# radhofan/Fairify

Hardware: AMD Instinct MI355X
Metric: % partitions verified + partitions/sec on AC suite at 1/2/4/8 MI355X (higher is better)
Workload: dtype fp32

## Files before the change

### fairify_amd/csrc/args.h

```cpp
#pragma once
#include "common.h"

#define FA_MAX_PA 8
#define FA_MAX_RA 8
#define FA_CMAX_PA 8
#define FA_MAX_SPLIT 6

struct BoundArgs {
  const float* flat;
  const float* lo;
  const float* hi;
  const uint8_t* dead_in;
  int R;
  int symbolic;
  int G;
  int stride;
  int wstride;
  int wfloats;
  float* out_lb;
  float* out_ub;
  float* Lc; float* L0; float* Le;
  float* Uc; float* U0; float* Ue;
  float* layer_lb;
  float* layer_ub;
  uint8_t* dead_out;
  int V;
  int npa;
  int pa_idx[FA_MAX_PA];
  const float* values;
  const int* node_part;
  const uint8_t* dead_part;
  int part_mod;
  unsigned long long fold;
  const int8_t* skip_status;
  const int* skip_part;
  int skip_signdef;
  const uint8_t* row_open;
  int open_mod;
  const int8_t* phase_in;
  uint8_t* infeas;
};

#define FA_MAX_ESC 4
struct EscSteps {
  int n;
  int budget[FA_MAX_ESC];
  int open[FA_MAX_ESC];
};

struct FwdArgs {
  const float* flat;
  const float* x;
  int B;
  const uint8_t* dead;
  float* out;
  int S;
};

struct AscentArgs {
  const float* flat;
  const float* lo;
  const float* hi;
  const float* x0;
  const float* f0;
  const int* q0;
  int P, K, iters;
  int V, npa;
  int pa_idx[FA_MAX_PA];
  const int64_t* values;
  int Pp;
  const int64_t* pairs;
  int nfree;
  int free_idx[64];
  uint8_t* found;
  float* wit_x;
  float* wit_xp;
  int S;
};

struct FalsifyArgs {
  const float* flat;
  const float* lo;
  const float* hi;
  const int64_t* pids;
  int P;
  int n_samples;
  int n_local;
  uint32_t seed;
  int V, npa;
  int pa_idx[FA_MAX_PA];
  const int64_t* values;
  int Pp;
  const int64_t* pairs;
  int walk_k, walk_steps;
  int K, iters;
  int nfree;
  int free_idx[64];
  uint8_t* found;
  float* wit_x;
  float* wit_xp;
  int8_t* how;
  int nra;
  int ra_idx[FA_MAX_RA];
  int tau;
  uint32_t dseed;
};

struct SimArgs {
  const float* flat;
  const float* lo;
  const float* hi;
  const int64_t* pids;
  int P;
  int n_samples;
  uint32_t seed;
  int V;
  int npa;
  int pa_idx[FA_MAX_PA];
  const int64_t* values;
  int Pp;
  const int64_t* pairs;
  int nra;
  int ra_idx[FA_MAX_RA];
  int tau;
  int* counts;
  uint8_t* found;
  float* wit_x;
  float* wit_xp;
  float* z0;
  int* keys;
  int split;
  int S;
  int regcount;
};

struct CertArgs {
  int Nn, n0, V, Pp, norient;
  const float *Lc, *L0, *Le, *Uc, *U0, *Ue;
  const float *Lcp, *L0p, *Lep, *Ucp, *U0p, *Uep;
  const float *olb, *oub, *olbp, *oubp;
  const float *xlo, *xhi, *xplo, *xphi;
  const int64_t* pairs;
  const int64_t* values;
  int npa;
  int pa_idx[FA_CMAX_PA];
  int nra;
  int ra_idx[FA_MAX_RA];
  float tau;
  const uint8_t* shared;
  float unit;
  float gmarg;
  float* gmin;
  float* tstar;
  uint8_t* open;
  float* score;
  int64_t* split_dim;
  float* cand_x;
  float* cand_xp;
  int64_t* cand_v;
  int64_t* cand_o;
  float* scores;
  uint8_t* leaf;
  int skip_closed;
  const int8_t* status;
  const int* part;
  int smear;
  const float* lay_lb;
  const float* lay_ub;
  int lay_N;
  const float* W0T;
  int n1;
};

struct SettleArgs {
  int P;
  int8_t* status;
  int* lvl_open;
  int* part_open;
  const int* part_nodes;
  int* nodes_start;
  int* prev_start;
  const int* counters_cur;
  int* counters_next;
  int* host_counts;
  int* pbudget;
  uint8_t* prob;
  int budget2;
  int max_open;
  EscSteps esc;
  int* done;
};

struct SplitArgs {
  int Nn, n0, relaxed, nra, V, Pp, norient;
  int ra_idx[FA_MAX_RA];
  float tau;
  const float *xlo, *xhi, *xplo, *xphi;
  const int* part;
  const uint8_t* open;
  const uint8_t* leaf;
  const float* scores;
  const float* cand_x;
  const float* cand_xp;
  const float* pe_lb;
  const float* pe_ub;
  const float *olb, *oub, *olbp, *oubp;
  const int64_t* pairs;
  const int64_t* values;
  int npa;
  int pa_idx[FA_CMAX_PA];
  const uint8_t* shared;
  int8_t* status;
  int* part_nodes;
  int* part_open;
  int* lvl_open;
  const int* nodes_start;
  const int* prev_start;
  int budget;
  const int* pbudget;
  uint8_t* prob;
  int budget2;
  int m;
  int target;
  float *oxlo, *oxhi, *oxplo, *oxphi;
  int* opart;
  int* count_out;
  int cap;
  float* cand_buf;
  int* cand_count;
  int cand_cap;
  SettleArgs settle;
};

struct BabInitArgs {
  int P, n_run, n0;
  const unsigned char* stage;
  int8_t* status;
  int *nodes, *open_left, *lvl_open, *nodes_start, *prev_start;
  int* part;
  float *xlo, *xhi, *xplo, *xphi;
  int nra;
  int ra_idx[FA_MAX_RA];
  float tau;
  int* counters;
  int* pbudget;
  uint8_t* prob;
  int budget;
};

#define FA_DECODE_MAX_DIMS 64
struct DecodeDesc {
  int n0;
  int radix[FA_DECODE_MAX_DIMS];
  long long div[FA_DECODE_MAX_DIMS];
  int chunk_off[FA_DECODE_MAX_DIMS];
  float base_lo[FA_DECODE_MAX_DIMS];
  float base_hi[FA_DECODE_MAX_DIMS];
};

struct CrownPhaseArgs {
  const float* flat;
  const float* lo;
  const float* hi;
  int R;
  const int8_t* phase;
  const float* layer_lb;
  const float* layer_ub;
  const uint8_t* infeas;
  float* out_lb;
  float* out_ub;
  float *Lc, *L0, *Le, *Uc, *U0, *Ue;
  int* split;
  float* score;
  float* low;
  const int8_t* skip_status;
  const int* skip_part;
};

struct ReluLevelArgs {
  int Nn, n0, nh;
  int npa;
  int pa_idx[FA_CMAX_PA];
  const int64_t* pairs;
  const float* values;
  int neg_from;
  const int* part;
  const int* pair;
  const float* xlo;
  const float* xhi;
  const int8_t* phase;
  float* rlo;
  float* rhi;
  int* rpart;
  const float* olb;
  const float* oub;
  const uint8_t* infeas;
  const float *Lc, *L0, *Le, *Uc, *U0, *Ue;
  const int* split;
  uint8_t* open;
  int* choice;
  int* idim;
  float* cpts;
  const float* pe_lb;
  const float* pe_ub;
  int8_t* status;
  int* part_nodes;
  const int* nodes_start;
  int budget;
  int* opart;
  int* opair;
  float* oxlo;
  float* oxhi;
  int8_t* ophase;
  int* count_out;
  int cap;
  float* cand_buf;
  int* cand_count;
  int cand_cap;
  float unit;
  float gmarg;
  int nra;
  int ra_idx[FA_MAX_RA];
  float tau;
  const float* xplo;
  const float* xphi;
  float* oxplo;
  float* oxphi;
};

struct BetaArgs {
  const float* flat;
  const float* wt;
  int R;
  int npa;
  int pa_idx[FA_MAX_PA];
  const float* lo;
  const float* hi;
  const float* va;
  const float* vb;
  const float* LBA;
  const float* UBA;
  const float* LBB;
  const float* UBB;
  const int8_t* phA;
  const int8_t* phB;
  float* par;
  float* t;
  float* scratch;
  int iters;
  float lr_a, lr_b, lr_t, decay;
  int lookahead;
  int beta_pos;
  int stall;
  int pgap;
  int wpb;
  int wt_lds;
  double* bound;
  int* split;
  float* xstar;
  float* binit;
  unsigned long long ramask;
  const float* plo;
  const float* phi;
  float* xpstar;
  float* gtie;
  float tau;
  const int8_t* osg;
  const uint8_t* skip;
  int ph_stride;
  int feas;
  const float* pgsum;
  const float* pgn;
  float* fpar;
  float* fgt;
  double* fval;
};

struct BetaPoolArgs {
  int N;
  int n0, nh, nn;
  int npa;
  int pa_idx[FA_MAX_PA];
  int nra;
  int ra_idx[FA_MAX_RA];
  float tau;
  int leaf;
  int warm_beta;
  int count;
  const int* part; const int* tree; const int8_t* osg;
  const float* lo; const float* hi; const float* plo; const float* phi;
  const float* va; const float* vb;
  float* LBA; float* UBA; float* LBB; float* UBB;
  const int8_t* ph; const float* par; const float* t; const float* gt;
  int8_t* status; int* part_nodes; int budget;
  int* tree_cnt;
  uint8_t* skip;
  float* rlo; float* rhi; int* rpart;
  const float* lay_lb; const float* lay_ub;
  const uint8_t* infeas;
  const double* bound; const int* split; const float* xstar; const float* xpstar; const float* binit;
  float* cpts;
  const float* pe_lb; const float* pe_ub;
  int* opart; int* otree; int8_t* oosg;
  float* olo; float* ohi; float* oplo; float* ophi; float* ova; float* ovb;
  float* oLBA; float* oUBA; float* oLBB; float* oUBB;
  int8_t* oph; float* opar; float* ot; float* ogt;
  int* count_out; int cap;
  int* nan_count;
  int* diag;
  int root;
  float* cand_buf; int* cand_count; int cand_cap;
};

#define FA_RATE_SLOTS 32
#define FA_RATE_MAX_V 32
#define FA_RATE_MAX_E 32
struct RateArgs {
  const float* flat;
  const float* lo;
  const float* hi;
  const int64_t* pids;
  int P;
  int n_samples;
  uint32_t seed;
  int V;
  int npa;
  int pa_idx[FA_MAX_PA];
  const int64_t* values;
  int Pp;
  const int64_t* pairs;
  int nra;
  int ra_idx[FA_MAX_RA];
  int tau;
  int E;
  int* flips;
  int* amb;
  int* amb_idx;
  int split;
};

#define FA_COUNT_MAX_VOL 65536
struct EnumArgs {
  const float* flat;
  const float* lo;
  const float* hi;
  int L;
  int V;
  int npa;
  int pa_idx[FA_MAX_PA];
  const int64_t* values;
  int Pp;
  const int64_t* pairs;
  int nra;
  int ra_idx[FA_MAX_RA];
  int tau;
  int E;
  int max_vol;
  int* cert;
  int* amb;
  int* amb_idx;
  int blocks;
};

struct CountArgs {
  int N, n0, V;
  int npa;
  int pa_idx[FA_MAX_PA];
  int nra;
  int ra_idx[FA_MAX_RA];
  float tau;
  const float* lo;
  const float* hi;
  const float* values;
  float* rlo;
  float* rhi;
  float* plo;
  float* phi;
  const int* part;
  const float *lx, *ux;
  const float *lxp, *uxp;
  int Pp;
  const int64_t* pairs;
  const float* score;
  long long leaf_points;
  uint8_t* code;
  long long* fair;
  long long* unfair;
  int* child_cnt;
  float* olo;
  float* ohi;
  int* opart;
  int cap;
  float* leaf_lo;
  float* leaf_hi;
  int* leaf_part;
  int leaf_cap;
  int* counters;
};
```

### fairify_amd/csrc/bab.hip

```cpp
#include <stdlib.h>

#include <algorithm>

#include "args.h"

#define ST_UNKNOWN 0
#define ST_SAT 1
#define ST_UNSAT 2
#define ST_RUNNING 3
#define ST_STOPPING 4

__device__ __forceinline__ void fa_stop(const SplitArgs& a, int p) { a.status[p] = ST_STOPPING; }

template <class DIMS>
__device__ __forceinline__ void fa_child_dim(const SplitArgs& a, const float* xl, const float* xh, const float* pl,
                                             const float* ph, const DIMS& dims, int m, int c, int d, float& lo,
                                             float& hi, float& plo, float& phi) {
  lo = xl[d]; hi = xh[d]; plo = pl[d]; phi = ph[d];
  for (int j = 0; j < m; ++j) {
    const int dd = dims[j];
    const bool up = (c >> j) & 1;
    if (dd == d) {
      const float mid = floorf(0.5f * (xl[d] + xh[d]));
      if (up) lo = mid + 1.f; else hi = mid;
      if (a.relaxed && a.shared[d]) { plo = lo; phi = hi; }
    } else if (dd == a.n0 + d) {
      const float mid = floorf(0.5f * (pl[d] + ph[d]));
      if (up) plo = mid + 1.f; else phi = mid;
    }
  }
  if (a.relaxed)
    for (int k = 0; k < a.nra; ++k)
      if (a.ra_idx[k] == d) {
        plo = fmaxf(plo, lo - a.tau);
        phi = fminf(phi, hi + a.tau);
        lo = fmaxf(lo, plo - a.tau);
        hi = fminf(hi, phi + a.tau);
      }
}

struct FaPackedDims {
  unsigned long long v;
  __device__ __forceinline__ int operator[](int j) const { return (int)((v >> (7 * j)) & 127ull); }
};

__device__ __forceinline__ void fa_wave_argmax(float& s, int& d) {
#pragma unroll
  for (int o = 32; o > 0; o >>= 1) {
    const float s2 = __shfl_xor(s, o);
    const int d2 = __shfl_xor(d, o);
    if (s2 > s || (s2 == s && d2 < d)) { s = s2; d = d2; }
  }
}

__device__ __forceinline__ void fa_group_argmax(float& s, int& d) {
#pragma unroll
  for (int o = 8; o > 0; o >>= 1) {
    const float s2 = __shfl_xor(s, o);
    const int d2 = __shfl_xor(d, o);
    if (s2 > s || (s2 == s && d2 < d)) { s = s2; d = d2; }
  }
}

__device__ __forceinline__ void fa_settle_counters(const SettleArgs& s) {
  const int c0 = __hip_atomic_load(&s.counters_cur[0], __ATOMIC_RELAXED, __HIP_MEMORY_SCOPE_AGENT);
  const int c1 = __hip_atomic_load(&s.counters_cur[1], __ATOMIC_RELAXED, __HIP_MEMORY_SCOPE_AGENT);
  __hip_atomic_store(&s.host_counts[0], c0, __ATOMIC_RELAXED, __HIP_MEMORY_SCOPE_SYSTEM);
  __hip_atomic_store(&s.host_counts[1], c1, __ATOMIC_RELAXED, __HIP_MEMORY_SCOPE_SYSTEM);
  s.counters_next[0] = 0;
  s.counters_next[1] = 0;
}

__device__ __forceinline__ void fa_settle_part(const SettleArgs& s, int p) {
  const int8_t st = s.status[p];
  if (st == ST_STOPPING) {
    s.status[p] = ST_UNKNOWN;
    if (s.part_open) s.part_open[p] = s.lvl_open[p];
  } else if (s.prob && s.prob[p] && st == ST_RUNNING) {
    const int cur = s.pbudget[p];
    int k = 0;
    while (k < s.esc.n && s.esc.budget[k] <= cur) ++k;
    const int thr = k == 0 ? s.max_open : s.esc.open[k - 1];
    if (s.lvl_open[p] <= thr) {
      s.pbudget[p] = k < s.esc.n ? s.esc.budget[k] : s.budget2;
    } else {
      s.status[p] = ST_UNKNOWN;
      if (s.part_open) s.part_open[p] = s.lvl_open[p];
    }
  }
  if (s.prob) s.prob[p] = 0;
  s.lvl_open[p] = 0;
  s.prev_start[p] = s.nodes_start[p];
  s.nodes_start[p] = s.part_nodes[p];
}

struct FaSplitPlan {
  unsigned long long fmask;
  unsigned long long dims;
  int m;
  int nchild;
  int ncand;
  int leaf;
  int part;
};

__device__ __forceinline__ bool fa_leaf_poss(const SplitArgs& a, int n, int t) {
  const int o = t / a.Pp, q = t - o * a.Pp;
  const size_t ri = (size_t)n * a.V + (int)a.pairs[2 * q], rj = (size_t)n * a.V + (int)a.pairs[2 * q + 1];
  return (o == 0) ? (a.olb[ri] < 0.f && a.oubp[rj] > 0.f) : (a.oub[ri] > 0.f && a.olbp[rj] < 0.f);
}

__device__ __forceinline__ int fa_wave_incl_scan(int v, int lane) {
#pragma unroll
  for (int o = 1; o < 64; o <<= 1) {
    const int u = __shfl_up(v, o);
    if (lane >= o) v += u;
  }
  return v;
}

#define FA_SPLIT_WAVES 8
#define FA_SPLIT_NPW 8
#define FA_SPLIT_NB (FA_SPLIT_WAVES * FA_SPLIT_NPW)
struct FaSplitLds {
  FaSplitPlan plan[FA_SPLIT_NB];
  int child_off[FA_SPLIT_NB], cand_off[FA_SPLIT_NB];
  int part[FA_SPLIT_NB], ns[FA_SPLIT_NB], ws[FA_SPLIT_NB], bud[FA_SPLIT_NB];
  float pe[FA_SPLIT_NB][4];
  int8_t st[FA_SPLIT_NB];
  uint8_t open[FA_SPLIT_NB], leaf[FA_SPLIT_NB];
  int last;
};

__device__ __forceinline__ void fa_split_fetch(const SplitArgs& a, FaSplitLds& sh, int nb) {
  if (threadIdx.x >= nb && threadIdx.x < FA_SPLIT_NB) sh.plan[threadIdx.x] = FaSplitPlan{0ull, 0ull, 0, 0, 0, 0, -1};
  if (threadIdx.x < nb) {
    const int t = threadIdx.x;
    const int n = blockIdx.x * nb + t;
    uint8_t op = 0;
    int p = 0;
    if (n < a.Nn) {
      op = a.open[n];
      p = a.part[n];
      sh.leaf[t] = a.leaf[n];
      sh.pe[t][0] = a.pe_lb[n];
      sh.pe[t][1] = a.pe_ub[n];
      sh.pe[t][2] = a.pe_lb[a.Nn + n];
      sh.pe[t][3] = a.pe_ub[a.Nn + n];
    }
    sh.open[t] = op;
    sh.part[t] = p;
    if (op) {
      sh.st[t] = a.status[p];
      sh.ns[t] = a.nodes_start[p];
      sh.ws[t] = a.nodes_start[p] - a.prev_start[p];
      sh.bud[t] = a.pbudget ? a.pbudget[p] : a.budget;
    }
  }
  __syncthreads();
}

__device__ __forceinline__ void fa_split_reserve(const SplitArgs& a, FaSplitLds& sh) {
  const int lane = threadIdx.x & 63;
  __syncthreads();
  if (threadIdx.x < 64) {
    const int c = sh.plan[lane].nchild, q = sh.plan[lane].ncand;
    const int ci = fa_wave_incl_scan(c, lane), qi = fa_wave_incl_scan(q, lane);
    int cb = 0, qb = 0;
    if (lane == 63) {
      if (ci) cb = atomicAdd(a.count_out, ci);
      if (qi) qb = atomicAdd(a.cand_count, qi);
    }
    cb = __shfl(cb, 63);
    qb = __shfl(qb, 63);
    sh.child_off[lane] = cb + ci - c;
    sh.cand_off[lane] = qb + qi - q;
    const int p = sh.plan[lane].part;
    const int o = p >= 0 ? 1 : 0;
    const int oi = fa_wave_incl_scan(o, lane);
    const int pprev = __shfl_up(p, 1), pnext = __shfl_down(p, 1);
    const unsigned long long heads = __ballot(lane == 0 || pprev != p);
    const bool tail = lane == 63 || pnext != p;
    const int h = 63 - __clzll(heads & (lane == 63 ? ~0ull : ((2ull << lane) - 1ull)));
    const int ci_b = __shfl(ci, h > 0 ? h - 1 : 0), oi_b = __shfl(oi, h > 0 ? h - 1 : 0);
    if (tail && p >= 0) {
      const int so = oi - (h > 0 ? oi_b : 0), sc = ci - (h > 0 ? ci_b : 0);
      if (so && a.lvl_open) atomicAdd(&a.lvl_open[p], so);
      if (sc) atomicAdd(&a.part_nodes[p], sc);
    }
  }
  __syncthreads();
}

__device__ __forceinline__ void fa_split_settle_tail(const SplitArgs& a, FaSplitLds& sh) {
  if (a.settle.P > 0) {
    __threadfence();
    __syncthreads();
    if (threadIdx.x == 0) sh.last = atomicAdd(a.settle.done, 1) == (int)gridDim.x - 1;
    __syncthreads();
    if (sh.last) {
      __threadfence();
      if (threadIdx.x == 0) fa_settle_counters(a.settle);
      for (int p = threadIdx.x; p < a.settle.P; p += blockDim.x) fa_settle_part(a.settle, p);
      if (threadIdx.x == 0) *a.settle.done = 0;
    }
  }
}

__device__ __forceinline__ void fa_split_write_leaf(const SplitArgs& a, int n, int p, int t, int slot) {
  const int n0 = a.n0;
  if (slot >= a.cand_cap) {
    fa_stop(a, p);
    return;
  }
  const float* xl = a.xlo + (size_t)n * n0;
  const float* xpl = a.relaxed ? a.xplo + (size_t)n * n0 : xl;
  const int o = t / a.Pp, q = t - o * a.Pp;
  const int vi = (int)a.pairs[2 * q], vj = (int)a.pairs[2 * q + 1];
  float* cbuf = a.cand_buf + (size_t)slot * (2 * n0 + 1);
  for (int d = 0; d < n0; ++d) {
    cbuf[d] = xl[d];
    cbuf[n0 + d] = xpl[d];
  }
  for (int k = 0; k < a.npa; ++k) {
    cbuf[a.pa_idx[k]] = (float)a.values[vi * a.npa + k];
    cbuf[n0 + a.pa_idx[k]] = (float)a.values[vj * a.npa + k];
  }
  cbuf[2 * n0] = __int_as_float(p);
}

template <int W>
__device__ __forceinline__ void fa_split_write_inner(const SplitArgs& a, const FaSplitPlan& pl, int n, int p, int slot,
                                                     int off, int li) {
  const int n0 = a.n0;
  const float* xl = a.xlo + (size_t)n * n0;
  const float* xh = a.xhi + (size_t)n * n0;
  const float* xpl = a.relaxed ? a.xplo + (size_t)n * n0 : xl;
  const float* xph = a.relaxed ? a.xphi + (size_t)n * n0 : xh;
  if (pl.ncand) {
    if (slot < a.cand_cap) {
      float* cbuf = a.cand_buf + (size_t)slot * (2 * n0 + 1);
      for (int d = li; d < 2 * n0 + 1; d += W)
        cbuf[d] = d < n0 ? a.cand_x[(size_t)n * n0 + d]
                         : (d < 2 * n0 ? a.cand_xp[(size_t)n * n0 + d - n0] : __int_as_float(p));
    }
  }
  if (pl.nchild == 0) return;
  if (off + pl.nchild > a.cap) {
    if (li == 0) fa_stop(a, p);
    const int lim = a.cap - off;
    for (int e = li; e < lim * n0; e += W) {
      const int r = e / n0, d = e - r * n0;
      const size_t o = (size_t)(off + r) * n0 + d;
      a.oxlo[o] = xl[d];
      a.oxhi[o] = xh[d];
      if (a.relaxed) { a.oxplo[o] = xpl[d]; a.oxphi[o] = xph[d]; }
    }
    for (int r = li; r < lim; r += W) a.opart[off + r] = p;
    return;
  }
  const FaPackedDims dims{pl.dims};
  for (int c = li; c < (1 << pl.m); c += W)
    if ((pl.fmask >> c) & 1ull) a.opart[off + __popcll(pl.fmask & ((1ull << c) - 1ull))] = p;
  const int dense = (pl.fmask & (pl.fmask + 1ull)) == 0ull;
  for (int e = li; e < pl.nchild * n0; e += W) {
    const int r = e / n0, d = e - r * n0;
    int c = r;
    if (!dense) {
      unsigned long long mm = pl.fmask;
      for (int t = 0; t < r; ++t) mm &= mm - 1ull;
      c = __ffsll((long long)mm) - 1;
    }
    float lo, hi, plo, phi;
    fa_child_dim(a, xl, xh, xpl, xph, dims, pl.m, c, d, lo, hi, plo, phi);
    const size_t o = (size_t)(off + r) * n0 + d;
    a.oxlo[o] = lo;
    a.oxhi[o] = hi;
    if (a.relaxed) {
      a.oxplo[o] = plo;
      a.oxphi[o] = phi;
    }
  }
}

__global__ void __launch_bounds__(64 * FA_SPLIT_WAVES) fa_split_kernel(SplitArgs a, int npw) {
  __shared__ FaSplitLds sh;
  const int lane = threadIdx.x & 63;
  const int wave = threadIdx.x >> 6;
  const int n0 = a.n0;
  const int npair = a.norient * a.Pp;
  const int nb = FA_SPLIT_WAVES * npw;
  fa_split_fetch(a, sh, nb);
  for (int i = 0; i < npw; ++i) {
    const int loc = wave * npw + i;
    const int n = blockIdx.x * nb + loc;
    FaSplitPlan pl{0ull, 0ull, 0, 0, 0, 0, -1};
    do {
      if (n >= a.Nn || !sh.open[loc]) break;
      const int p = sh.part[loc];
      const int8_t s0 = sh.st[loc];
      if (s0 != ST_RUNNING && s0 != ST_STOPPING) break;
      if (sh.leaf[loc]) {
        pl.leaf = 1;
        for (int t0 = 0; t0 < npair; t0 += 64)
          pl.ncand += __popcll(__ballot(t0 + lane < npair && fa_leaf_poss(a, n, t0 + lane)));
        break;
      }
      pl.part = p;
      {
        const float lbx = sh.pe[loc][0], ubx = sh.pe[loc][1];
        const float lbp = sh.pe[loc][2], ubp = sh.pe[loc][3];
        pl.ncand = ((lbx < 0.f && ubp > 0.f) || (ubx > 0.f && lbp < 0.f)) ? 1 : 0;
      }
      const float* sc = a.scores + (size_t)n * 2 * n0;
      int mreq = 1;
      {
        const int mmax = a.m < FA_MAX_SPLIT ? a.m : FA_MAX_SPLIT;
        const int w = sh.ws[loc];
        while (mreq < mmax && ((long long)w << (mreq + 1)) <= (long long)a.target) ++mreq;
      }
      const int d0 = lane, d1 = lane + 64;
      float s0v = (d0 < 2 * n0) ? sc[d0] : -1.f;
      float s1v = (d1 < 2 * n0) ? sc[d1] : -1.f;
      if (!(s0v > -0.5f)) s0v = -1.f;
      if (!(s1v > -0.5f)) s1v = -1.f;
      int dims[FA_MAX_SPLIT];
      int m = 0;
      for (int j = 0; j < mreq; ++j) {
        float sv = s0v >= s1v ? s0v : s1v;
        int d = s0v >= s1v ? d0 : d1;
        if (sv <= -0.5f) d = 0x7fffffff;
        fa_wave_argmax(sv, d);
        if (sv <= -0.5f) break;
        dims[m++] = d;
        if (d == d0) s0v = -1.f;
        if (d == d1) s1v = -1.f;
      }
      if (m == 0) break;
      {
        const int bud = sh.bud[loc];
        if (sh.ns[loc] >= bud) {
          if (a.prob && bud < a.budget2) {
            if (lane == 0) a.prob[p] = 1;
          } else {
            if (lane == 0) fa_stop(a, p);
            break;
          }
        }
      }
      const int k = 1 << m;
      const float* xl = a.xlo + (size_t)n * n0;
      const float* xh = a.xhi + (size_t)n * n0;
      const float* xpl = a.relaxed ? a.xplo + (size_t)n * n0 : xl;
      const float* xph = a.relaxed ? a.xphi + (size_t)n * n0 : xh;
      bool ok = lane < k;
      if (a.relaxed && ok)
        for (int d = 0; d < n0; ++d) {
          float lo, hi, plo, phi;
          fa_child_dim(a, xl, xh, xpl, xph, dims, m, lane, d, lo, hi, plo, phi);
          ok = ok && lo <= hi && plo <= phi;
        }
      pl.fmask = __ballot(ok);
      pl.nchild = __popcll(pl.fmask);
      pl.m = m;
      for (int j = 0; j < m; ++j) pl.dims |= (unsigned long long)dims[j] << (7 * j);
    } while (false);
    if (lane == 0) sh.plan[loc] = pl;
  }
  fa_split_reserve(a, sh);
  for (int i = 0; i < npw; ++i) {
    const int loc = wave * npw + i;
    const int n = blockIdx.x * nb + loc;
    const FaSplitPlan pl = sh.plan[loc];
    if (pl.ncand == 0 && pl.nchild == 0) continue;
    const int p = sh.part[loc];
    if (pl.leaf) {
      int slot0 = sh.cand_off[loc];
      for (int t0 = 0; t0 < npair; t0 += 64) {
        const int t = t0 + lane;
        const bool poss = t < npair && fa_leaf_poss(a, n, t);
        const unsigned long long bm = __ballot(poss);
        if (poss) {
          const int slot = slot0 + __popcll(bm & ((1ull << lane) - 1ull));
          fa_split_write_leaf(a, n, p, t, slot);
        }
        slot0 += __popcll(bm);
      }
      continue;
    }
    fa_split_write_inner<64>(a, pl, n, p, sh.cand_off[loc], sh.child_off[loc], lane);
  }
  fa_split_settle_tail(a, sh);
}

#define FA_SPLIT_GPW 4
#define FA_SPLIT_NPP (FA_SPLIT_NB / (FA_SPLIT_WAVES * FA_SPLIT_GPW))
__global__ void __launch_bounds__(64 * FA_SPLIT_WAVES) fa_split_group_kernel(SplitArgs a, int npp) {
  __shared__ FaSplitLds sh;
  const int lane = threadIdx.x & 63;
  const int wave = threadIdx.x >> 6;
  const int gl = lane & 15, grp = lane >> 4;
  const int n0 = a.n0;
  const int npair = a.norient * a.Pp;
  const int nb = FA_SPLIT_WAVES * FA_SPLIT_GPW * npp;
  const int mmax = a.m < FA_MAX_SPLIT ? a.m : FA_MAX_SPLIT;
  fa_split_fetch(a, sh, nb);
  for (int i = 0; i < npp; ++i) {
    const int loc = (wave * npp + i) * FA_SPLIT_GPW + grp;
    const int n = blockIdx.x * nb + loc;
    FaSplitPlan pl{0ull, 0ull, 0, 0, 0, 0, -1};
    bool act = n < a.Nn && sh.open[loc];
    const int p = sh.part[loc];
    if (act) {
      const int8_t s0 = sh.st[loc];
      act = s0 == ST_RUNNING || s0 == ST_STOPPING;
    }
    const bool lf = act && sh.leaf[loc];
    if (__ballot(lf)) {
      for (int t0 = 0; t0 < npair; t0 += 16) {
        const unsigned long long bm = __ballot(lf && t0 + gl < npair && fa_leaf_poss(a, n, t0 + gl));
        pl.ncand += __popcll((bm >> (16 * grp)) & 0xffffull);
      }
    }
    pl.leaf = lf ? 1 : 0;
    const bool inner = act && !lf;
    int mreq = 1;
    float s0v = -1.f, s1v = -1.f;
    const int d0 = gl, d1 = gl + 16;
    if (inner) {
      pl.part = p;
      const float lbx = sh.pe[loc][0], ubx = sh.pe[loc][1];
      const float lbp = sh.pe[loc][2], ubp = sh.pe[loc][3];
      pl.ncand = ((lbx < 0.f && ubp > 0.f) || (ubx > 0.f && lbp < 0.f)) ? 1 : 0;
      const int w = sh.ws[loc];
      while (mreq < mmax && ((long long)w << (mreq + 1)) <= (long long)a.target) ++mreq;
      const float* sc = a.scores + (size_t)n * 2 * n0;
      if (d0 < 2 * n0) s0v = sc[d0];
      if (d1 < 2 * n0) s1v = sc[d1];
      if (!(s0v > -0.5f)) s0v = -1.f;
      if (!(s1v > -0.5f)) s1v = -1.f;
    }
    int m = 0;
    bool more = inner;
#pragma unroll
    for (int j = 0; j < FA_MAX_SPLIT; ++j) {
      float sv = s0v >= s1v ? s0v : s1v;
      int d = s0v >= s1v ? d0 : d1;
      if (sv <= -0.5f) d = 0x7fffffff;
      fa_group_argmax(sv, d);
      more = more && j < mreq && sv > -0.5f;
      if (more) {
        pl.dims |= (unsigned long long)d << (7 * j);
        m = j + 1;
        if (d == d0) s0v = -1.f;
        if (d == d1) s1v = -1.f;
      }
    }
    bool split = inner && m > 0;
    if (split) {
      const int bud = sh.bud[loc];
      if (sh.ns[loc] >= bud) {
        if (a.prob && bud < a.budget2) {
          if (gl == 0) a.prob[p] = 1;
        } else {
          if (gl == 0) fa_stop(a, p);
          split = false;
        }
      }
    }
    {
      const FaPackedDims dims{pl.dims};
      const float* xl = a.xlo + (size_t)n * n0;
      const float* xh = a.xhi + (size_t)n * n0;
      const float* xpl = a.relaxed ? a.xplo + (size_t)n * n0 : xl;
      const float* xph = a.relaxed ? a.xphi + (size_t)n * n0 : xh;
      unsigned long long fmask = 0ull;
      for (int c0 = 0; c0 < (1 << (mmax > 1 ? mmax : 1)); c0 += 16) {
        const int c = c0 + gl;
        bool ok = split && c < (1 << m);
        if (a.relaxed && ok)
          for (int d = 0; d < n0; ++d) {
            float lo, hi, plo, phi;
            fa_child_dim(a, xl, xh, xpl, xph, dims, m, c, d, lo, hi, plo, phi);
            ok = ok && lo <= hi && plo <= phi;
          }
        const unsigned long long bm = __ballot(ok);
        fmask |= ((bm >> (16 * grp)) & 0xffffull) << c0;
      }
      if (split) {
        pl.fmask = fmask;
        pl.nchild = __popcll(fmask);
        pl.m = m;
      } else {
        pl.dims = 0ull;
      }
    }
    if (gl == 0) sh.plan[loc] = pl;
  }
  fa_split_reserve(a, sh);
  for (int i = 0; i < npp; ++i) {
    const int loc = (wave * npp + i) * FA_SPLIT_GPW + grp;
    const int n = blockIdx.x * nb + loc;
    const FaSplitPlan pl = sh.plan[loc];
    const bool any = pl.ncand != 0 || pl.nchild != 0;
    if (!__ballot(any)) continue;
    const int p = sh.part[loc];
    const bool lf = any && pl.leaf;
    if (__ballot(lf)) {
      int slot0 = sh.cand_off[loc];
      for (int t0 = 0; t0 < npair; t0 += 16) {
        const int t = t0 + gl;
        const bool poss = lf && t < npair && fa_leaf_poss(a, n, t);
        const unsigned long long bm = (__ballot(poss) >> (16 * grp)) & 0xffffull;
        if (poss) fa_split_write_leaf(a, n, p, t, slot0 + __popcll(bm & ((1ull << gl) - 1ull)));
        slot0 += __popcll(bm);
      }
    }
    if (any && !pl.leaf) fa_split_write_inner<16>(a, pl, n, p, sh.cand_off[loc], sh.child_off[loc], gl);
  }
  fa_split_settle_tail(a, sh);
}

__global__ void fa_bab_init_kernel(BabInitArgs a) {
  const int tid = blockIdx.x * FA_THREADS + threadIdx.x;
  const int nth = gridDim.x * FA_THREADS;
  const int8_t* st = reinterpret_cast<const int8_t*>(a.stage);
  const int* run = reinterpret_cast<const int*>(a.stage + ((a.P + 3) & ~3));
  const float* lo = reinterpret_cast<const float*>(run + a.n_run);
  const float* hi = lo + (size_t)a.n_run * a.n0;
  for (int p = tid; p < a.P; p += nth) {
    a.status[p] = st[p];
    a.nodes[p] = 0;
    a.open_left[p] = 0;
    a.lvl_open[p] = 0;
    a.nodes_start[p] = 0;
    a.prev_start[p] = -1;
    if (a.pbudget) a.pbudget[p] = a.budget;
    if (a.prob) a.prob[p] = 0;
  }
  for (int i = tid; i < a.n_run; i += nth) a.part[i] = run[i];
  const size_t ne = (size_t)a.n_run * a.n0;
  for (size_t e = tid; e < ne; e += nth) {
    a.xlo[e] = lo[e];
    a.xhi[e] = hi[e];
    if (a.xplo) {
      const int d = (int)(e % a.n0);
      bool r = false;
      for (int k = 0; k < a.nra; ++k) r |= a.ra_idx[k] == d;
      a.xplo[e] = r ? lo[e] - a.tau : lo[e];
      a.xphi[e] = r ? hi[e] + a.tau : hi[e];
    }
  }
  if (tid < 5) a.counters[tid] = 0;
}

__global__ void fa_bab_finish_kernel(int P, const int8_t* status, const int* nodes, const int* open_left, int* out) {
  const int p = blockIdx.x * FA_THREADS + threadIdx.x;
  if (p >= P) return;
  out[p] = status[p];
  out[P + p] = nodes[p];
  out[2 * P + p] = open_left[p];
}

__global__ void fa_mark_unknown_kernel(const int* part, int n, int8_t* status) {
  const int i = blockIdx.x * FA_THREADS + threadIdx.x;
  if (i >= n) return;
  const int p = part[i];
  if (status[p] == ST_RUNNING || status[p] == ST_STOPPING) status[p] = ST_UNKNOWN;
}

__global__ void fa_settle_kernel(SettleArgs s) {
  const int p = blockIdx.x * FA_THREADS + threadIdx.x;
  if (p == 0) fa_settle_counters(s);
  if (p < s.P) fa_settle_part(s, p);
}

__global__ void fa_set_status_kernel(const int* idx, int n, int8_t* status, int8_t v) {
  const int i = blockIdx.x * FA_THREADS + threadIdx.x;
  if (i < n) status[idx[i]] = v;
}

extern "C" int fa_split_launch(SplitArgs a, hipStream_t stream) {
  if (a.Nn <= 0) return 0;
  if (a.nra > FA_MAX_RA || a.npa > FA_CMAX_PA || a.n0 > 64) return -3;
  if (2 * a.n0 <= 32) {
    const char* e = getenv("FAIRIFY_SPLIT_GROUPS");
    if (!(e && *e == '0')) {
      int npp = FA_SPLIT_NPP;
      while (npp > 1 && (a.Nn + FA_SPLIT_WAVES * FA_SPLIT_GPW * npp - 1) / (FA_SPLIT_WAVES * FA_SPLIT_GPW * npp) < 1024)
        npp >>= 1;
      const int nbg = FA_SPLIT_WAVES * FA_SPLIT_GPW * npp;
      hipLaunchKernelGGL(fa_split_group_kernel, dim3((a.Nn + nbg - 1) / nbg), dim3(64 * FA_SPLIT_WAVES), 0, stream, a,
                         npp);
      return (int)hipGetLastError();
    }
  }
  int npw = FA_SPLIT_NPW;
  while (npw > 1 && (a.Nn + FA_SPLIT_WAVES * npw - 1) / (FA_SPLIT_WAVES * npw) < 1024) npw >>= 1;
  const int nb = FA_SPLIT_WAVES * npw;
  hipLaunchKernelGGL(fa_split_kernel, dim3((a.Nn + nb - 1) / nb), dim3(64 * FA_SPLIT_WAVES), 0, stream, a, npw);
  return (int)hipGetLastError();
}

extern "C" int fa_mark_unknown_launch(const int* part, int n, int8_t* status, hipStream_t stream) {
  if (n <= 0) return 0;
  hipLaunchKernelGGL(fa_mark_unknown_kernel, dim3((n + FA_THREADS - 1) / FA_THREADS), dim3(FA_THREADS), 0, stream,
                     part, n, status);
  return (int)hipGetLastError();
}

extern "C" int fa_set_status_launch(const int* idx, int n, int8_t* status, int8_t v, hipStream_t stream) {
  if (n <= 0) return 0;
  hipLaunchKernelGGL(fa_set_status_kernel, dim3((n + FA_THREADS - 1) / FA_THREADS), dim3(FA_THREADS), 0, stream, idx,
                     n, status, v);
  return (int)hipGetLastError();
}

extern "C" int fa_settle_launch(SettleArgs s, hipStream_t stream) {
  const int n = s.P > 0 ? s.P : 1;
  hipLaunchKernelGGL(fa_settle_kernel, dim3((n + FA_THREADS - 1) / FA_THREADS), dim3(FA_THREADS), 0, stream, s);
  return (int)hipGetLastError();
}

extern "C" int fa_bab_init_launch(BabInitArgs a, hipStream_t stream) {
  if (a.nra > FA_MAX_RA) return -3;
  const long long work = std::max<long long>(std::max(a.P, a.n_run), (long long)a.n_run * a.n0);
  const int blocks = (int)std::min<long long>((work + FA_THREADS - 1) / FA_THREADS + 1, 4096);
  hipLaunchKernelGGL(fa_bab_init_kernel, dim3(blocks), dim3(FA_THREADS), 0, stream, a);
  return (int)hipGetLastError();
}

extern "C" int fa_bab_finish_launch(int P, const int8_t* status, const int* nodes, const int* open_left, int* out,
                                    hipStream_t stream) {
  if (P <= 0) return 0;
  hipLaunchKernelGGL(fa_bab_finish_kernel, dim3((P + FA_THREADS - 1) / FA_THREADS), dim3(FA_THREADS), 0, stream, P,
                     status, nodes, open_left, out);
  return (int)hipGetLastError();
}
```

### fairify_amd/csrc/bab_runtime.cpp

```cpp
#include <hip/hip_runtime.h>
#include <pybind11/numpy.h>
#include <pybind11/pybind11.h>
#include <pybind11/stl.h>

#include <algorithm>
#include <chrono>
#include <cmath>
#include <cstring>
#include <stdexcept>
#include <utility>
#include <vector>

#include "runtime_host.h"

namespace py = pybind11;

extern "C" int fa_certify_launch(CertArgs a, hipStream_t stream);
extern "C" int fa_split_launch(SplitArgs a, hipStream_t stream);
extern "C" int fa_mark_unknown_launch(const int* part, int n, int8_t* status, hipStream_t stream);
extern "C" int fa_settle_launch(SettleArgs s, hipStream_t stream);
extern "C" int fa_crown_launch(const NetDesc& net, BoundArgs a, hipStream_t stream);
extern "C" int fa_refine_launch(const NetDesc& net, BoundArgs a, hipStream_t stream);
extern "C" int fa_backward_launch(const NetDesc& net, BoundArgs a, hipStream_t stream);
extern "C" int fa_refine_crown_launch(const NetDesc& net, BoundArgs a, hipStream_t stream);
extern "C" int fa_bab_init_launch(BabInitArgs a, hipStream_t stream);
extern "C" int fa_bab_finish_launch(int P, const int8_t* status, const int* nodes, const int* open_left, int* out,
                                    hipStream_t stream);

const NetDesc& fa_net_desc(py::handle net);

namespace {

using fa_mem::DevBuf;
using fa_rt::ck;
using fa_rt::ckl;

bool point_skip_closed() {
  static const bool v = [] {
    const char* e = getenv("FAIRIFY_POINT_SKIP_CLOSED");
    return !(e && e[0] == '0');
  }();
  return v;
}

bool cert_skip_closed() {
  static const bool v = [] {
    const char* e = getenv("FAIRIFY_CERT_SKIP_CLOSED");
    return !(e && e[0] == '0');
  }();
  return v;
}

bool fuse_settle() {
  static const bool v = [] {
    const char* e = getenv("FAIRIFY_FUSE_SETTLE");
    return e && e[0] == '1';
  }();
  return v;
}

bool skip_signdef() {
  static const bool v = [] {
    const char* e = getenv("FAIRIFY_REFINE_SKIP_SIGNDEF");
    return !(e && e[0] == '0');
  }();
  return v;
}

}

class BabRuntime {
 public:
  BabRuntime(py::handle net, uintptr_t flat, std::vector<int> pa, std::vector<float> values_f,
             std::vector<int64_t> values_i, std::vector<int64_t> pairs, std::vector<int> ra, float tau,
             std::vector<uint8_t> shared, int capacity, int batch_nodes, int cand_cap, double unit, bool crown,
             int split_target, int refine, bool smear, py::object keep)
      : net_(fa_net_desc(net)),
        flat_((const float*)flat),
        keep_(std::move(keep)),
        pa_(std::move(pa)),
        ra_(std::move(ra)),
        tau_(tau),
        cap_(capacity),
        batch_(batch_nodes),
        cand_cap_(cand_cap),
        unit_(unit),
        crown_(crown),
        refine_(crown ? refine : 0),
        smear_(smear),
        split_target_(std::max(2, split_target)),
        sink_(net_.dims[0]) {
    n0_ = net_.dims[0];
    npa_ = (int)pa_.size();
    if (npa_ == 0 || npa_ > FA_CMAX_PA || (int)ra_.size() > FA_MAX_RA) throw std::invalid_argument("bad PA/RA");
    V_ = (int)(values_i.size() / npa_);
    Pp_ = (int)(pairs.size() / 2);
    relaxed_ = !ra_.empty() && tau_ > 0;
    norient_ = relaxed_ ? 2 : 1;
    if ((int)shared.size() != n0_) throw std::invalid_argument("shared mask size");
    vals_f_.ensure(values_f.size());
    vals_i_.ensure(values_i.size());
    pairs_.ensure(pairs.size());
    shared_.ensure(shared.size());
    ck(hipMemcpy(vals_f_.p, values_f.data(), values_f.size() * sizeof(float), hipMemcpyHostToDevice), "cp");
    ck(hipMemcpy(vals_i_.p, values_i.data(), values_i.size() * sizeof(int64_t), hipMemcpyHostToDevice), "cp");
    ck(hipMemcpy(pairs_.p, pairs.data(), pairs.size() * sizeof(int64_t), hipMemcpyHostToDevice), "cp");
    ck(hipMemcpy(shared_.p, shared.data(), shared.size(), hipMemcpyHostToDevice), "cp");
    pool_[0] = pool_[1] = 0;
    const size_t R = (size_t)batch_ * V_;
    for (int s = 0; s < (relaxed_ ? 2 : 1); ++s) form_[s].ensure(R, n0_, net_.n_neurons, crown_ || smear_);
    const size_t Q = (size_t)Pp_ * norient_;
    gmin_.ensure(batch_ * Q);
    tstar_.ensure(batch_ * Q);
    open_.ensure(batch_);
    leaf_.ensure(batch_);
    score_.ensure(batch_);
    split_.ensure(batch_);
    cv_.ensure(batch_);
    co_.ensure(batch_);
    cand_.ensure((size_t)2 * batch_ * n0_);
    scores_.ensure((size_t)batch_ * 2 * n0_);
    pe_lb_.ensure(2 * (size_t)batch_);
    pe_ub_.ensure(2 * (size_t)batch_);
    sink_.ensure_cand(cand_cap_, kCandFloor);
    counters_.ensure(5);
    exact_ = fa_rt::make_exact(net_, flat_, pa_, relaxed_ ? ra_ : std::vector<int>(), tau_);
    if (smear_ && n0_ > 32) smear_ = false;
    if (smear_) {
      const int nm = n0_ <= 16 ? 16 : 32, n1 = net_.dims[1];
      std::vector<float> wt((size_t)n1 * nm, 0.f);
      for (int j = 0; j < n1; ++j)
        for (int i = 0; i < n0_; ++i)
          wt[(size_t)j * nm + i] = (float)std::fabs(exact_.w[(size_t)net_.w_off[0] + (size_t)i * n1 + j]);
      w0t_.ensure(wt.size());
      ck(hipMemcpy(w0t_.p, wt.data(), wt.size() * sizeof(float), hipMemcpyHostToDevice), "cp w0t");
    }
  }

  void set_fuse_settle(bool v) { fuse_settle_ = v; }

  py::tuple solve(py::array_t<float, py::array::c_style | py::array::forcecast> lo,
                  py::array_t<float, py::array::c_style | py::array::forcecast> hi,
                  py::array_t<int8_t, py::array::c_style | py::array::forcecast> status0, int budget,
                  double time_budget, uintptr_t dead_part, py::object confirm, uintptr_t stream_i,
                  bool native_exact, int budget2, int max_w, std::vector<std::pair<int, int>> esc_steps) {
    const bool inline_esc = budget2 > budget && max_w > 0;
    EscSteps esc{};
    for (const auto& bo : esc_steps)
      if (bo.first > (esc.n ? esc.budget[esc.n - 1] : budget) && bo.first < budget2 && esc.n < FA_MAX_ESC) {
        esc.budget[esc.n] = bo.first;
        esc.open[esc.n] = bo.second;
        ++esc.n;
      }
    hipStream_t st = (hipStream_t)stream_i;
    const auto t0 = std::chrono::steady_clock::now();
    const int P = (int)lo.shape(0);
    if (lo.ndim() != 2 || lo.shape(1) != n0_ || hi.shape(0) != P || status0.shape(0) != P)
      throw std::invalid_argument("solve: shape mismatch");
    status_.ensure(P);
    nodes_.ensure(P);
    open_left_.ensure(P);
    lvl_open_.ensure(P);
    nodes_start_.ensure(P);
    prev_start_.ensure(P);
    if (inline_esc) {
      pbudget_.ensure(P);
      prob_.ensure(P);
    }
    int slot = 0;
    const int8_t* hstatus = status0.data();
    std::vector<int> run;
    for (int p = 0; p < P; ++p)
      if (hstatus[p] == 3) run.push_back(p);
    if ((int)run.size() > cap_) throw std::invalid_argument("more partitions than pool capacity");
    ensure_pool(0, std::max<long long>((long long)run.size(), 1));
    const size_t nrun = run.size();
    const size_t st_bytes = (size_t)((P + 3) & ~3) + nrun * sizeof(int) + 2 * nrun * n0_ * sizeof(float);
    hstage_.ensure(st_bytes);
    stage_.ensure(st_bytes);
    {
      unsigned char* h = hstage_.p;
      std::memcpy(h, hstatus, P);
      int* hr = reinterpret_cast<int*>(h + ((P + 3) & ~3));
      std::memcpy(hr, run.data(), nrun * sizeof(int));
      float* hl = reinterpret_cast<float*>(hr + nrun);
      float* hh = hl + nrun * n0_;
      for (size_t i = 0; i < nrun; ++i)
        for (int d = 0; d < n0_; ++d) {
          hl[i * n0_ + d] = lo.data()[(size_t)run[i] * n0_ + d];
          hh[i * n0_ + d] = hi.data()[(size_t)run[i] * n0_ + d];
        }
    }
    ck(hipMemcpyAsync(stage_.p, hstage_.p, st_bytes, hipMemcpyHostToDevice, st), "cp stage");
    {
      BabInitArgs ia{};
      ia.P = P; ia.n_run = (int)nrun; ia.n0 = n0_;
      ia.stage = stage_.p;
      ia.status = status_.p; ia.nodes = nodes_.p; ia.open_left = open_left_.p; ia.lvl_open = lvl_open_.p;
      ia.nodes_start = nodes_start_.p; ia.prev_start = prev_start_.p;
      ia.part = part_[0].p; ia.xlo = lo_[0].p; ia.xhi = hi_[0].p;
      ia.xplo = relaxed_ ? plo_[0].p : nullptr; ia.xphi = relaxed_ ? phi_[0].p : nullptr;
      ia.nra = relaxed_ ? (int)ra_.size() : 0;
      for (int k = 0; k < ia.nra; ++k) ia.ra_idx[k] = ra_[k];
      ia.tau = tau_;
      ia.counters = counters_.p;
      ia.pbudget = inline_esc ? pbudget_.p : nullptr;
      ia.prob = inline_esc ? prob_.p : nullptr;
      ia.budget = budget;
      ckl(fa_bab_init_launch(ia, st), "bab_init");
    }
    int cur = 0;
    int n_in = (int)nrun;
    fa_exact::Witnesses wit(P, n0_, lo.data(), hi.data());
    hcount_.reset();
    int levels = 0, launches = 0, cand_overflow = 0;
    long long total_nodes = 0;
    bool timed_out = false;
    {
    py::gil_scoped_release nogil;
    while (n_in > 0) {
      const double el = std::chrono::duration<double>(std::chrono::steady_clock::now() - t0).count();
      if (el > time_budget) {
        ckl(fa_mark_unknown_launch(part_[cur].p, n_in, status_.p, st), "mark");
        timed_out = true;
        break;
      }
      int* cnt = counters_.p + 2 * slot;
      const int nxt = cur ^ 1;
      ensure_pool(nxt, 2LL * n_in + (long long)split_target_ * std::min(P, n_in));
      sink_.ensure_cand((long long)n_in * std::max(1, Pp_ * norient_), kCandFloor);
      SettleArgs se{};
      se.P = P; se.status = status_.p; se.lvl_open = lvl_open_.p; se.part_open = open_left_.p;
      se.part_nodes = nodes_.p; se.nodes_start = nodes_start_.p; se.prev_start = prev_start_.p;
      se.counters_cur = cnt; se.counters_next = counters_.p + 2 * (slot ^ 1); se.host_counts = hcount_.host_ptr();
      se.pbudget = inline_esc ? pbudget_.p : nullptr; se.prob = inline_esc ? prob_.p : nullptr;
      se.budget2 = budget2; se.max_open = max_w; se.esc = esc;
      se.done = counters_.p + 4;
      bool settled = false;
      for (int s = 0; s < n_in; s += batch_) {
        const int nb = std::min(batch_, n_in - s);
        const float* blo = lo_[cur].p + (size_t)s * n0_;
        const float* bhi = hi_[cur].p + (size_t)s * n0_;
        const float* bplo = relaxed_ ? plo_[cur].p + (size_t)s * n0_ : blo;
        const float* bphi = relaxed_ ? phi_[cur].p + (size_t)s * n0_ : bhi;
        const int* bpart = part_[cur].p + s;
        launch_bounds(blo, bhi, bpart, nb, 0, dead_part, st);
        if (relaxed_) launch_bounds(bplo, bphi, bpart, nb, 1, dead_part, st);
        const int sx = relaxed_ ? 1 : 0;
        CertArgs c{};
        c.Nn = nb; c.n0 = n0_; c.V = V_; c.Pp = Pp_; c.norient = norient_;
        const fa_rt::FormBufs &fx = form_[0], &fp = form_[sx];
        c.Lc = fx.Lc.p; c.L0 = fx.L0.p; c.Le = fx.Le.p; c.Uc = fx.Uc.p; c.U0 = fx.U0.p; c.Ue = fx.Ue.p;
        c.Lcp = fp.Lc.p; c.L0p = fp.L0.p; c.Lep = fp.Le.p; c.Ucp = fp.Uc.p; c.U0p = fp.U0.p; c.Uep = fp.Ue.p;
        c.olb = fx.olb.p; c.oub = fx.oub.p; c.olbp = fp.olb.p; c.oubp = fp.oub.p;
        c.xlo = blo; c.xhi = bhi; c.xplo = bplo; c.xphi = bphi;
        c.pairs = pairs_.p; c.values = vals_i_.p; c.npa = npa_;
        for (int k = 0; k < npa_; ++k) c.pa_idx[k] = pa_[k];
        c.nra = relaxed_ ? (int)ra_.size() : 0;
        for (int k = 0; k < c.nra; ++k) c.ra_idx[k] = ra_[k];
        c.tau = tau_;
        c.shared = shared_.p;
        c.unit = (float)unit_;
        c.gmarg = fa_rt::gamma_up(2 * n0_ + 4, unit_);
        c.gmin = gmin_.p; c.tstar = tstar_.p;
        c.open = open_.p; c.score = score_.p; c.split_dim = split_.p;
        c.cand_x = cand_.p; c.cand_xp = cand_.p + (size_t)nb * n0_;
        c.cand_v = cv_.p; c.cand_o = co_.p;
        c.scores = scores_.p; c.leaf = leaf_.p;
        if (cert_skip_closed()) { c.skip_closed = 1; c.status = status_.p; c.part = bpart; }
        if (smear_ && !relaxed_) {
          c.smear = 1;
          c.lay_lb = fx.lay_lb.p; c.lay_ub = fx.lay_ub.p; c.lay_N = net_.n_neurons;
          c.W0T = w0t_.p; c.n1 = net_.dims[1];
        }
        ckl(fa_certify_launch(c, st), "certify");
        fa_rt::screen_points(net_, flat_, cand_.p, 2 * nb, pe_lb_.p, pe_ub_.p, st, bpart, nb,
                             (const uint8_t*)dead_part, point_skip_closed() ? open_.p : nullptr, nb);
        SplitArgs sa{};
        sa.Nn = nb; sa.n0 = n0_; sa.relaxed = relaxed_ ? 1 : 0; sa.nra = relaxed_ ? (int)ra_.size() : 0;
        for (int k = 0; k < sa.nra; ++k) sa.ra_idx[k] = ra_[k];
        sa.V = V_; sa.Pp = Pp_; sa.norient = norient_; sa.tau = tau_;
        sa.xlo = blo; sa.xhi = bhi; sa.xplo = bplo; sa.xphi = bphi; sa.part = bpart;
        sa.open = open_.p; sa.leaf = leaf_.p; sa.scores = scores_.p;
        sa.cand_x = c.cand_x; sa.cand_xp = c.cand_xp; sa.pe_lb = pe_lb_.p; sa.pe_ub = pe_ub_.p;
        sa.olb = c.olb; sa.oub = c.oub; sa.olbp = c.olbp; sa.oubp = c.oubp;
        sa.pairs = pairs_.p; sa.values = vals_i_.p; sa.npa = npa_;
        for (int k = 0; k < npa_; ++k) sa.pa_idx[k] = pa_[k];
        sa.shared = shared_.p;
        sa.status = status_.p; sa.part_nodes = nodes_.p; sa.part_open = open_left_.p; sa.lvl_open = lvl_open_.p;
        sa.nodes_start = nodes_start_.p;
        sa.prev_start = prev_start_.p;
        sa.budget = budget; sa.m = FA_MAX_SPLIT; sa.target = split_target_;
        sa.pbudget = inline_esc ? pbudget_.p : nullptr;
        sa.prob = inline_esc ? prob_.p : nullptr;
        sa.budget2 = budget2;
        sa.oxlo = lo_[nxt].p; sa.oxhi = hi_[nxt].p;
        sa.oxplo = relaxed_ ? plo_[nxt].p : nullptr; sa.oxphi = relaxed_ ? phi_[nxt].p : nullptr;
        sa.opart = part_[nxt].p; sa.count_out = cnt; sa.cap = pool_[nxt];
        sa.cand_buf = sink_.records(); sa.cand_count = cnt + 1; sa.cand_cap = sink_.cand_alloc_;
        if (s + nb >= n_in && fuse_settle_) {
          sa.settle = se;
          settled = true;
        }
        ckl(fa_split_launch(sa, st), "split");
        launches += (relaxed_ ? 2 : 1) * (refine_ == 2 ? 1 : 2) + 3;
      }
      if (!settled) {
        ckl(fa_settle_launch(se, st), "settle");
        ++launches;
      }
      ck(hipStreamSynchronize(st), "sync");
      slot ^= 1;
      total_nodes += n_in;
      const int n_out = std::min(hcount_.children(), pool_[nxt]);
      const int n_cand_all = hcount_.candidates();
      const int n_cand = std::min(n_cand_all, sink_.cand_alloc_);
      if (n_cand_all > sink_.cand_alloc_) ++cand_overflow;
      ++levels;
      if (n_cand > 0)
        sink_.confirm_candidates(n_cand, wit, native_exact ? &exact_ : nullptr, confirm, status_.p, st);
      cur = nxt;
      n_in = n_out;
    }
    }
    out_.ensure((size_t)3 * P);
    hout_.ensure((size_t)3 * P * sizeof(int));
    ckl(fa_bab_finish_launch(P, status_.p, nodes_.p, open_left_.p, out_.p, st), "bab_finish");
    ck(hipMemcpyAsync(hout_.p, out_.p, (size_t)3 * P * sizeof(int), hipMemcpyDeviceToHost, st), "cp out");
    ck(hipStreamSynchronize(st), "sync");
    const int* hres = reinterpret_cast<const int*>(hout_.p);
    py::array_t<int8_t> status_out(P);
    py::array_t<int64_t> nodes_out(P), open_out(P);
    for (int p = 0; p < P; ++p) {
      int8_t v = (int8_t)hres[p];
      if (wit.got[p]) v = 1;
      else if (v == 3) v = timed_out ? 0 : 2;
      status_out.mutable_data()[p] = v;
      nodes_out.mutable_data()[p] = hres[P + p];
      open_out.mutable_data()[p] = (v == 0) ? hres[2 * P + p] : 0;
    }
    const double el = std::chrono::duration<double>(std::chrono::steady_clock::now() - t0).count();
    py::dict stats;
    stats["levels"] = levels;
    stats["launches"] = launches;
    stats["cand_overflow_levels"] = cand_overflow;
    stats["nodes"] = total_nodes;
    stats["time"] = el;
    stats["timed_out"] = timed_out;
    py::array_t<int64_t> ax({P, n0_}), axp({P, n0_});
    std::memcpy(ax.mutable_data(), wit.cex_x.data(), sizeof(int64_t) * wit.cex_x.size());
    std::memcpy(axp.mutable_data(), wit.cex_xp.data(), sizeof(int64_t) * wit.cex_xp.size());
    stats["open_left"] = open_out;
    return py::make_tuple(status_out, ax, axp, nodes_out, stats);
  }

 private:
  void launch_bounds(const float* lo, const float* hi, const int* part, int nb, int slot, uintptr_t dead_part,
                     hipStream_t st) {
    BoundArgs b{};
    b.flat = flat_;
    b.lo = lo;
    b.hi = hi;
    b.R = nb * V_;
    b.symbolic = 1;
    form_[slot].fill(b);
    b.V = V_;
    b.npa = npa_;
    for (int k = 0; k < npa_; ++k) b.pa_idx[k] = pa_[k];
    b.values = vals_f_.p;
    if (dead_part) {
      b.node_part = part;
      b.dead_part = (const uint8_t*)dead_part;
    }
    b.skip_status = status_.p;
    b.skip_part = part;
    if (refine_ == 2) {
      if (smear_) { b.layer_lb = form_[slot].lay_lb.p; b.layer_ub = form_[slot].lay_ub.p; }
      const int rc = fa_backward_launch(net_, b, st);
      if (rc == 0) return;
      if (rc != -1) ckl(rc, "backward");
      refine_ = 1;
    }
    if (crown_ || smear_) {
      b.layer_lb = form_[slot].lay_lb.p;
      b.layer_ub = form_[slot].lay_ub.p;
    }
    ckl(fa_bounds_launch(net_, b, st), "bounds");
    if (refine_ == 1) {
      b.skip_signdef = (!relaxed_ && npa_ == 1 && Pp_ == V_ * (V_ - 1) && skip_signdef()) ? 1 : 0;
      const int rc = fa_refine_crown_launch(net_, b, st);
      if (rc == 0) return;
      if (rc != -1) ckl(rc, "refine");
      refine_ = 0;
    }
    if (crown_) {
      const int rc = fa_crown_launch(net_, b, st);
      if (rc == -1) crown_ = false;
      else ckl(rc, "crown");
    }
  }

  void ensure_pool(int i, long long need) {
    const int want = (int)std::min<long long>(std::max<long long>(need, 1), cap_);
    if (want <= pool_[i]) return;
    const int n = fa_rt::grow_to(pool_[i], want, 1 << 16, cap_);
    const size_t cn = (size_t)n * n0_;
    lo_[i].ensure(cn);
    hi_[i].ensure(cn);
    part_[i].ensure(n);
    if (relaxed_) {
      plo_[i].ensure(cn);
      phi_[i].ensure(cn);
    }
    pool_[i] = n;
  }

  NetDesc net_;
  const float* flat_;
  py::object keep_;
  fa_exact::ExactChecker exact_;
  std::vector<int> pa_, ra_;
  float tau_;
  int cap_, batch_, cand_cap_;
  static constexpr int kCandFloor = 1 << 16;
  int pool_[2] = {0, 0};
  double unit_;
  bool crown_ = false;
  int refine_ = 0;
  bool smear_ = false;
  bool fuse_settle_ = fuse_settle();
  int split_target_ = 256;
  int n0_ = 0, npa_ = 0, V_ = 0, Pp_ = 0, norient_ = 1;
  bool relaxed_ = false;
  DevBuf<float> vals_f_, w0t_;
  DevBuf<int64_t> vals_i_, pairs_;
  DevBuf<uint8_t> shared_;
  DevBuf<float> lo_[2], hi_[2], plo_[2], phi_[2];
  DevBuf<int> part_[2];
  fa_rt::FormBufs form_[2];
  DevBuf<float> gmin_, tstar_, score_, cand_, scores_, pe_lb_, pe_ub_;
  DevBuf<uint8_t> open_, leaf_;
  DevBuf<int64_t> split_, cv_, co_;
  DevBuf<int> counters_, nodes_, open_left_, lvl_open_, nodes_start_, prev_start_, out_, pbudget_;
  DevBuf<int8_t> status_;
  DevBuf<uint8_t> prob_;
  DevBuf<unsigned char> stage_;
  fa_rt::LevelCounters hcount_;
  fa_mem::HostBuf hstage_, hout_;
  fa_rt::CandSink sink_;
};

void register_bab(py::module& m) {
  py::class_<BabRuntime>(m, "BabRuntime")
      .def(py::init<py::handle, uintptr_t, std::vector<int>, std::vector<float>, std::vector<int64_t>,
                    std::vector<int64_t>, std::vector<int>, float, std::vector<uint8_t>, int, int, int, double, bool,
                    int, int, bool, py::object>(),
           py::arg("net"), py::arg("flat"), py::arg("pa"), py::arg("values_f"), py::arg("values_i"),
           py::arg("pairs"), py::arg("ra"), py::arg("tau"), py::arg("shared"), py::arg("capacity"),
           py::arg("batch_nodes"), py::arg("cand_cap"), py::arg("unit"), py::arg("crown") = true,
           py::arg("split_target") = 256, py::arg("refine") = 0, py::arg("smear") = false, py::arg("keep") = py::none())
      .def("set_fuse_settle", &BabRuntime::set_fuse_settle, py::arg("on"))
      .def("solve", &BabRuntime::solve, py::arg("lo"), py::arg("hi"), py::arg("status"), py::arg("budget"),
           py::arg("time_budget"), py::arg("dead_part"), py::arg("confirm"), py::arg("stream"),
           py::arg("native_exact") = false, py::arg("budget2") = 0, py::arg("max_w") = 0,
           py::arg("esc_steps") = std::vector<std::pair<int, int>>{});
}
```

### fairify_amd/csrc/bindings.cpp

```cpp
#include <hip/hip_runtime.h>
#include <pybind11/pybind11.h>
#include <pybind11/stl.h>

#include <algorithm>
#include <cmath>
#include <cstring>
#include <cstdint>
#include <stdexcept>
#include <vector>

#include "kwargs.h"
#include "runtime_host.h"

extern "C" int fa_bounds_launch(const NetDesc& net, BoundArgs args, hipStream_t stream);
extern "C" int fa_crown_phase_launch(const NetDesc& net, CrownPhaseArgs a, hipStream_t stream);
extern "C" size_t fa_crown_phase_bytes(const NetDesc& net);
extern "C" int fa_point_try_launch(const NetDesc& net, BoundArgs a, hipStream_t stream);
extern "C" int fa_forward_launch(const NetDesc& net, FwdArgs a, hipStream_t stream);
extern "C" int fa_sim_launch(const NetDesc& net, SimArgs a, hipStream_t stream);
extern "C" int fa_sim_shaped(const NetDesc& net);
extern "C" int fa_rate_launch(const NetDesc& net, RateArgs a, hipStream_t stream);
extern "C" int fa_count_enum_launch(const NetDesc& net, EnumArgs a, hipStream_t stream);
extern "C" int fa_count_rows_launch(CountArgs a, hipStream_t stream);
extern "C" int fa_count_level_launch(CountArgs a, hipStream_t stream);
extern "C" int fa_ascent_launch(const NetDesc& net, AscentArgs a, hipStream_t stream);
extern "C" int fa_certify_launch(CertArgs a, hipStream_t stream);
extern "C" int fa_falsify_launch(const NetDesc& net, FalsifyArgs a, hipStream_t stream);
extern "C" int fa_prune_masks_launch(const NetDesc& net, int P, const int* counts, const float* ub, int ub_stride,
                                     const uint8_t* sym_dead, uint8_t* code, int* cnt, hipStream_t stream);
extern "C" int fa_heuristic_launch(const NetDesc& net, int Pu, const int64_t* rows, const float* lb, const float* ub,
                                   int stride, const uint8_t* code, double q50, double qlo, double qhi, uint8_t* hnew,
                                   uint8_t* hmerged, int* hcnt, hipStream_t stream);
extern "C" int fa_agree_launch(const NetDesc& net, const float* flat, int Pm, const int64_t* rows, const float* lo,
                               const float* hi, const int64_t* pids, const uint8_t* dead, int S, uint32_t seed,
                               int* agree, hipStream_t stream);

extern "C" int fa_decode_launch(const DecodeDesc& d, const int64_t* ids, int P, const float* chunk_lo,
                                const float* chunk_hi, float* lo, float* hi, hipStream_t stream);
extern "C" int fa_trace_marker_launch(int tag, int* sink, hipStream_t stream);
extern "C" int fa_beta_launch(const NetDesc& nd, BetaArgs a, hipStream_t stream);
extern "C" int fa_beta_config(const NetDesc& nd, int* wpb, int* wtl, size_t* bytes);
extern "C" int fa_beta_opt16_fits(const NetDesc& nd);
extern "C" size_t fa_beta_opt16_scratch_floats(const NetDesc& nd, int R);
extern "C" int fa_beta_opt16_launch(const NetDesc& nd, BetaArgs a, float* pgsum, float* pgn, hipStream_t stream);
extern "C" int fa_beta_level16_launch(const NetDesc& nd, BetaArgs a, hipStream_t stream);
extern "C" int fa_beta_opt16_feas_launch(const NetDesc& nd, BetaArgs a, hipStream_t stream);
extern "C" int fa_beta_feas16_launch(const NetDesc& nd, BetaArgs a, hipStream_t stream);
extern "C" int fa_knn_launch(const float* X, int n, int d, int k, int* idx, float* dist, hipStream_t stream);
extern "C" int fa_actdiff_launch(const NetDesc& net, const float* flat, const float* x, const float* xp, int npairs,
                                 float* sum_out, hipStream_t stream);
extern "C" int fa_pack_masks_launch(const uint8_t* src, int P, int N, int stride, int sel, uint8_t* out, int NB,
                                    unsigned long long* hash, hipStream_t stream);

template <typename T>
static T* P(uintptr_t p) { return reinterpret_cast<T*>(p); }

using fa_rt::gamma_up;

struct Net {
  NetDesc d;
  explicit Net(const std::vector<int>& dims, double unit) {
    if (dims.size() < 2 || dims.size() > FA_MAX_LAYERS + 1) throw std::invalid_argument("bad layer count");
    std::memset(&d, 0, sizeof(d));
    d.n_layers = (int)dims.size() - 1;
    int off = 0, noff = 0, mw = 0, mws = 0;
    for (size_t i = 0; i < dims.size(); ++i) {
      d.dims[i] = dims[i];
      mw = std::max(mw, dims[i]);
    }
    for (int l = 0; l < d.n_layers; ++l) {
      d.w_off[l] = off;
      off += dims[l] * dims[l + 1];
      d.b_off[l] = off;
      off += dims[l + 1];
      d.neuron_off[l] = noff;
      noff += dims[l + 1];
      mws = std::max(mws, dims[l] * dims[l + 1]);
      d.g_gemm[l] = gamma_up(2 * dims[l] + 1, unit);
      d.g_fwd[l] = gamma_up(dims[l] + 1, unit);
    }
    d.n_neurons = noff;
    d.n_hidden = noff - dims.back();
    d.max_width = mw;
    d.max_wsize = mws;
    d.unit = (float)unit;
    d.g_conc = gamma_up(dims[0] + 1, unit);
    d.g_one = gamma_up(1, unit);
    n_params = off;
    d.wperm_off = (off + 3) & ~3;
    int wp = 0;
    for (int l = 0; l < d.n_layers; ++l) wp += ((dims[l] + 15) / 16) * ((dims[l + 1] + 15) / 16) * 256;
    for (int l = 0; l < d.n_layers; ++l) wp += dims[l + 1];
    d.wperm_floats = (wp + 3) & ~3;
    total_floats = d.wperm_off + d.wperm_floats;
    d.pack_g = 1;
    if (d.n_layers >= 2 && dims[0] <= 16 && mw <= 16) {
      int mh = 0;
      for (int l = 1; l < d.n_layers; ++l) mh = std::max(mh, dims[l]);
      d.pack_g = mh <= 4 ? 4 : (mh <= 8 ? 2 : 1);
    }
    d.pack_off = total_floats;
    d.pack_floats = 0;
    if (d.pack_g > 1) {
      d.pack_floats = d.pack_g * 256 + (d.n_layers - 1) * 256 + d.n_layers * 16;
      total_floats += d.pack_floats;
    }
    d.wback_off = total_floats;
    int wb = 0;
    for (int l = 0; l < d.n_layers; ++l) wb += ((dims[l] + 15) / 16) * ((dims[l + 1] + 15) / 16) * 256;
    d.wback_floats = wb;
    total_floats += wb;
  }
  int n_params;
  int total_floats;
};

const NetDesc& fa_net_desc(py::handle h) { return h.cast<const Net&>().d; }
void register_bab(py::module& m);
void register_relu(py::module& m);
void register_beta(py::module& m);
extern "C" int fa_crown_launch(const NetDesc& net, BoundArgs a, hipStream_t stream);
extern "C" int fa_refine_launch(const NetDesc& net, BoundArgs a, hipStream_t stream);
extern "C" int fa_backward_launch(const NetDesc& net, BoundArgs a, hipStream_t stream);
extern "C" int fa_refine_crown_launch(const NetDesc& net, BoundArgs a, hipStream_t stream);
void register_csv(py::module& m);

using fa_rt::ckl;

static hipStream_t finish(Kw& k) {
  const hipStream_t s = reinterpret_cast<hipStream_t>(k.u64("stream"));
  k.done();
  return s;
}

static int dims(Kw& k, const char* key, int* idx, size_t cap, const char* too_many) {
  const std::vector<int> v = k.ints(key);
  if (v.size() > cap) throw std::invalid_argument(too_many);
  std::copy(v.begin(), v.end(), idx);
  return (int)v.size();
}

enum { OUT = 1, FORMS = 2, LAYERS = 4 };
template <typename A>
static A row_args(Kw& k, int req, const char* lo = "lo", const char* hi = "hi") {
  auto p = [&](const char* key, int group) { return (req & group) ? k.need<float>(key) : k.ptr<float>(key); };
  A a{};
  a.flat = k.need<const float>("flat");
  a.lo = k.need<const float>(lo);
  a.hi = k.need<const float>(hi);
  a.R = k.i("R");
  a.out_lb = p("out_lb", OUT);
  a.out_ub = p("out_ub", OUT);
  a.Lc = p("Lc", FORMS); a.L0 = p("L0", FORMS); a.Le = p("Le", FORMS);
  a.Uc = p("Uc", FORMS); a.U0 = p("U0", FORMS); a.Ue = p("Ue", FORMS);
  a.layer_lb = p("layer_lb", LAYERS);
  a.layer_ub = p("layer_ub", LAYERS);
  return a;
}
static BoundArgs bound_args(Kw& k, int req, const char* lo = "lo", const char* hi = "hi") {
  BoundArgs a = row_args<BoundArgs>(k, req, lo, hi);
  a.dead_in = k.ptr<const uint8_t>("dead_in");
  return a;
}

template <typename A>
static void fill_query(A& a, Kw& k, const char* too_many) {
  a.flat = k.need<const float>("flat");
  a.lo = k.need<const float>("lo");
  a.hi = k.need<const float>("hi");
  a.P = k.i("P");
  a.V = k.i("V");
  a.npa = dims(k, "pa", a.pa_idx, FA_MAX_PA, too_many);
  a.values = k.ptr<const int64_t>("values");
  a.Pp = k.i("Pp");
  a.pairs = k.ptr<const int64_t>("pairs");
}
template <typename A>
static void fill_samples(A& a, Kw& k, const char* too_many) {
  a.pids = k.need<const int64_t>("pids");
  a.n_samples = k.i("n_samples");
  a.seed = (uint32_t)k.u64("seed");
  a.nra = dims(k, "ra", a.ra_idx, FA_MAX_RA, too_many);
  a.tau = k.i("tau");
}
template <typename A>
static void fill_ascent(A& a, Kw& k, const char* too_many) {
  a.K = k.i("K");
  a.iters = k.i("iters");
  a.nfree = dims(k, "free", a.free_idx, 64, too_many);
  a.found = k.need<uint8_t>("found");
  a.wit_x = k.need<float>("wit_x");
  a.wit_xp = k.need<float>("wit_xp");
}

static BetaArgs beta_args(const Net& net, Kw& k) {
  BetaArgs a;
  std::memset(&a, 0, sizeof(a));
  a.flat = k.need<const float>("flat");
  a.wt = k.ptr<const float>("wt");
  a.R = k.i("R");
  a.npa = dims(k, "pa", a.pa_idx, FA_MAX_PA, "beta_level: too many PA dims");
  for (int q = 0; q < a.npa; ++q)
    if (a.pa_idx[q] < 0 || a.pa_idx[q] >= net.d.dims[0] || (q && a.pa_idx[q] <= a.pa_idx[q - 1]))
      throw std::invalid_argument("beta_level: PA dims must be increasing input indices");
  a.lo = k.need<const float>("lo");
  a.hi = k.need<const float>("hi");
  a.va = k.need<const float>("va");
  a.vb = k.need<const float>("vb");
  a.LBA = k.need<const float>("LBA");
  a.UBA = k.need<const float>("UBA");
  a.LBB = k.need<const float>("LBB");
  a.UBB = k.need<const float>("UBB");
  a.phA = k.need<const int8_t>("phA");
  a.phB = k.need<const int8_t>("phB");
  a.par = k.need<float>("par");
  a.t = k.need<float>("t");
  a.scratch = k.need<float>("scratch");
  a.iters = k.i("iters");
  a.lr_a = k.f("lr_a");
  a.lr_b = k.f("lr_b");
  a.lr_t = k.f("lr_t");
  a.decay = k.f("decay");
  a.lookahead = k.i("lookahead", 0);
  a.beta_pos = k.i("beta_pos", 1);
  const int flags = k.i("flags", 0);
  a.stall = flags & 1;
  a.pgap = (flags >> 1) & 3;
  a.feas = (flags >> 3) & 1;
  a.bound = k.ptr<double>("bound");
  a.split = k.ptr<int>("split");
  a.xstar = k.ptr<float>("xstar");
  a.binit = k.ptr<float>("binit");
  a.ramask = k.u64("ramask", 0);
  a.plo = k.ptr<const float>("plo");
  a.phi = k.ptr<const float>("phi");
  a.xpstar = k.ptr<float>("xpstar");
  a.gtie = k.ptr<float>("gtie");
  a.tau = k.f("tau", 0.f);
  a.osg = k.ptr<const int8_t>("osg");
  a.pgsum = k.ptr<const float>("pgsum");
  a.pgn = k.ptr<const float>("pgn");
  a.fpar = k.ptr<float>("fpar");
  a.fgt = k.ptr<float>("fgt");
  a.fval = k.ptr<double>("fval");
  if ((net.d.dims[0] < 64 && (a.ramask >> net.d.dims[0])) || (a.ramask && (!a.plo || !a.phi)))
    throw std::invalid_argument("beta_level: RA mask beyond the inputs or no x' box");
  return a;
}

PYBIND11_MODULE(_C, m) {
  m.doc() = "fairify_amd CDNA4 (gfx950) kernels";
  py::class_<Net>(m, "Net")
      .def(py::init<const std::vector<int>&, double>())
      .def_readonly("n_params", &Net::n_params)
      .def_readonly("total_floats", &Net::total_floats)
      .def_property_readonly("wperm_off", [](const Net& n) { return n.d.wperm_off; })
      .def_property_readonly("pack_g", [](const Net& n) { return n.d.pack_g; })
      .def_property_readonly("pack_off", [](const Net& n) { return n.d.pack_off; })
      .def_property_readonly("n_hidden", [](const Net& n) { return n.d.n_hidden; })
      .def_property_readonly("n_neurons", [](const Net& n) { return n.d.n_neurons; });

  m.def("bounds", [](const Net& net, py::kwargs kw) {
    Kw k("bounds", kw);
    const int symbolic = k.i("symbolic");
    BoundArgs a = bound_args(k, symbolic ? OUT | FORMS : OUT);
    a.symbolic = symbolic;
    a.G = k.i("G", 0);
    a.dead_out = k.ptr<uint8_t>("dead_out");
    a.fold = k.u64("fold", 0);
    a.phase_in = k.ptr<const int8_t>("phase_in");
    a.infeas = k.ptr<uint8_t>("infeas");
    ckl(fa_bounds_launch(net.d, a, finish(k)), "bounds");
  });

  m.def("crown_phase", [](const Net& net, py::kwargs kw) {
    Kw k("crown_phase", kw);
    CrownPhaseArgs a = row_args<CrownPhaseArgs>(k, OUT | FORMS | LAYERS);
    a.phase = k.ptr<const int8_t>("phase");
    a.infeas = k.ptr<const uint8_t>("infeas");
    a.split = k.need<int>("split");
    a.score = k.need<float>("score");
    a.low = k.ptr<float>("low");
    const int rc = fa_crown_phase_launch(net.d, a, finish(k));
    if (rc != 0) throw std::runtime_error("crown_phase launch failed, code " + std::to_string(rc));
  });

  m.def("relu_fits", [](const Net& net) { return fa_crown_phase_bytes(net.d) > 0; });

  m.def("crown", [](const Net& net, py::kwargs kw) {
    Kw k("crown", kw);
    const BoundArgs a = bound_args(k, OUT | FORMS | LAYERS);
    ckl(fa_crown_launch(net.d, a, finish(k)), "crown");
  });

  m.def("refine", [](const Net& net, py::kwargs kw) {
    Kw k("refine", kw);
    BoundArgs a = bound_args(k, LAYERS);
    a.phase_in = k.ptr<const int8_t>("phase_in");
    a.infeas = k.ptr<uint8_t>("infeas");
    const int rc = fa_refine_launch(net.d, a, finish(k));
    if (rc < -1) throw std::runtime_error("refine launch failed, code " + std::to_string(rc));
    return rc;
  });
  m.def("refine_crown", [](const Net& net, py::kwargs kw) {
    Kw k("refine_crown", kw);
    const BoundArgs a = bound_args(k, OUT | FORMS | LAYERS);
    const int rc = fa_refine_crown_launch(net.d, a, finish(k));
    if (rc < -1) throw std::runtime_error("refine_crown launch failed, code " + std::to_string(rc));
    return rc;
  });
  m.def("backward_bounds", [](const Net& net, py::kwargs kw) {
    Kw k("backward_bounds", kw);
    const BoundArgs a = bound_args(k, OUT | FORMS);
    const int rc = fa_backward_launch(net.d, a, finish(k));
    if (rc < -1) throw std::runtime_error("backward_bounds launch failed, code " + std::to_string(rc));
    return rc;
  });

  m.def("point_bounds", [](const Net& net, py::kwargs kw) {
    Kw k("point_bounds", kw);
    BoundArgs a = bound_args(k, OUT, "x", "x");
    a.row_open = k.ptr<const uint8_t>("row_open");
    a.open_mod = k.i("open_mod", 0);
    if (a.row_open && a.open_mod <= 0) throw std::invalid_argument("point_bounds: row_open needs open_mod > 0");
    const hipStream_t stream = finish(k);
    const int rc = fa_point_try_launch(net.d, a, stream);
    if (rc < 0) ckl(-rc, "point_bounds");
    if (rc == 0) ckl(fa_bounds_launch(net.d, a, stream), "point_bounds(ibp)");
  });

  m.def("forward", [](const Net& net, uintptr_t flat, uintptr_t x, int B, uintptr_t dead, uintptr_t out,
                      uintptr_t stream) {
    FwdArgs a{};
    a.flat = P<const float>(flat);
    a.x = P<const float>(x);
    a.B = B;
    a.dead = P<const uint8_t>(dead);
    a.out = P<float>(out);
    ckl(fa_forward_launch(net.d, a, (hipStream_t)stream), "forward");
  });

  m.def("sim", [](const Net& net, py::kwargs kw) {
    Kw k("sim", kw);
    SimArgs a{};
    fill_query(a, k, "too many PA/RA dims");
    fill_samples(a, k, "too many PA/RA dims");
    a.counts = k.need<int>("counts");
    a.found = k.need<uint8_t>("found");
    a.wit_x = k.need<float>("wit_x");
    a.wit_xp = k.need<float>("wit_xp");
    a.z0 = k.ptr<float>("z0");
    a.keys = k.ptr<int>("keys");
    a.split = k.i("split");
    a.regcount = k.i("regcount");
    if (a.split < 1 || (a.split > 1 && !a.keys)) throw std::invalid_argument("sim: split > 1 needs a keys buffer");
    ckl(fa_sim_launch(net.d, a, finish(k)), "sim");
  });
  m.def("sim_shaped", [](const Net& net) { return fa_sim_shaped(net.d) != 0; });

  m.def("rate", [](const Net& net, py::kwargs kw) {
    Kw k("rate", kw);
    RateArgs a{};
    fill_query(a, k, "too many PA/RA dims");
    fill_samples(a, k, "too many PA/RA dims");
    a.E = k.i("E");
    a.flips = k.need<int>("flips");
    a.amb = k.need<int>("amb");
    a.amb_idx = k.need<int>("amb_idx");
    a.split = k.i("split");
    const int rc = fa_rate_launch(net.d, a, finish(k));
    if (rc == -3) throw std::invalid_argument("rate: shape not covered (layer > 160, inputs > 32, V > 32 or E > 32)");
    ckl(rc, "rate");
  });

  m.def("count_enum", [](const Net& net, py::kwargs kw) {
    Kw k("count_enum", kw);
    EnumArgs a{};
    a.flat = k.need<const float>("flat");
    a.lo = k.need<const float>("lo");
    a.hi = k.need<const float>("hi");
    a.L = k.i("L");
    a.V = k.i("V");
    a.npa = dims(k, "pa", a.pa_idx, FA_MAX_PA, "too many PA/RA dims");
    a.values = k.need<const int64_t>("values");
    a.Pp = k.i("Pp");
    a.pairs = k.ptr<const int64_t>("pairs");
    a.nra = dims(k, "ra", a.ra_idx, FA_MAX_RA, "too many PA/RA dims");
    a.tau = k.i("tau");
    a.E = k.i("E");
    a.max_vol = k.i("max_vol");
    a.cert = k.need<int>("cert");
    a.amb = k.need<int>("amb");
    a.amb_idx = k.need<int>("amb_idx");
    a.blocks = k.i("blocks");
    if (a.Pp > 0 && !a.pairs) throw py::type_error("count_enum() missing required keyword argument 'pairs'");
    const int rc = fa_count_enum_launch(net.d, a, finish(k));
    if (rc == -3)
      throw std::invalid_argument(
          "count_enum: shape not covered (layer > 160, inputs > 32, V > 32, E > 32 or leaf volume > 65536)");
    ckl(rc, "count_enum");
  });
  auto count_args = [](Kw& k) {
    CountArgs a{};
    a.N = k.i("N");
    a.n0 = k.i("n0");
    a.V = k.i("V");
    a.npa = dims(k, "pa", a.pa_idx, FA_MAX_PA, "too many PA/RA dims");
    a.lo = k.need<const float>("lo");
    a.hi = k.need<const float>("hi");
    return a;
  };
  m.def("count_rows", [count_args](py::kwargs kw) {
    Kw k("count_rows", kw);
    CountArgs a = count_args(k);
    a.nra = dims(k, "ra", a.ra_idx, FA_MAX_RA, "too many PA/RA dims");
    a.tau = k.f("tau");
    a.values = k.need<const float>("values");
    a.rlo = k.need<float>("rlo");
    a.rhi = k.need<float>("rhi");
    a.plo = k.ptr<float>("plo");
    a.phi = k.ptr<float>("phi");
    ckl(fa_count_rows_launch(a, finish(k)), "count_rows");
  });
  m.def("count_level", [count_args](py::kwargs kw) {
    Kw k("count_level", kw);
    CountArgs a = count_args(k);
    a.part = k.need<const int>("part");
    a.lx = k.need<const float>("lx");
    a.ux = k.need<const float>("ux");
    a.lxp = k.need<const float>("lxp");
    a.uxp = k.need<const float>("uxp");
    a.Pp = k.i("Pp");
    a.pairs = k.ptr<const int64_t>("pairs");
    a.score = k.need<const float>("score");
    a.leaf_points = (long long)k.u64("leaf_points");
    a.code = k.need<uint8_t>("code");
    a.fair = k.need<long long>("fair");
    a.unfair = k.need<long long>("unfair");
    a.child_cnt = k.need<int>("child_cnt");
    a.olo = k.need<float>("olo");
    a.ohi = k.need<float>("ohi");
    a.opart = k.need<int>("opart");
    a.cap = k.i("cap");
    a.leaf_lo = k.need<float>("leaf_lo");
    a.leaf_hi = k.need<float>("leaf_hi");
    a.leaf_part = k.need<int>("leaf_part");
    a.leaf_cap = k.i("leaf_cap");
    a.counters = k.need<int>("counters");
    if (a.Pp > 0 && !a.pairs) throw py::type_error("count_level() missing required keyword argument 'pairs'");
    ckl(fa_count_level_launch(a, finish(k)), "count_level");
  });

  m.def("ascent", [](const Net& net, py::kwargs kw) {
    Kw k("ascent", kw);
    AscentArgs a{};
    fill_query(a, k, "too many PA/free dims");
    fill_ascent(a, k, "too many PA/free dims");
    a.x0 = k.need<const float>("x0");
    a.f0 = k.need<const float>("f0");
    a.q0 = k.need<const int>("q0");
    const int rc = fa_ascent_launch(net.d, a, finish(k));
    if (rc == -1) return false;
    ckl(rc, "ascent");
    return true;
  });

  m.def("falsify", [](const Net& net, py::kwargs kw) {
    Kw k("falsify", kw);
    FalsifyArgs a{};
    fill_query(a, k, "too many PA/RA/free dims");
    fill_samples(a, k, "too many PA/RA/free dims");
    fill_ascent(a, k, "too many PA/RA/free dims");
    if (a.tau <= 0) {
      a.nra = 0;
      std::fill_n(a.ra_idx, FA_MAX_RA, 0);
    }
    a.n_local = k.i("n_local");
    a.walk_k = k.i("walk_k");
    a.walk_steps = k.i("walk_steps");
    a.how = k.need<int8_t>("how");
    a.dseed = (uint32_t)k.u64("dseed");
    const int rc = fa_falsify_launch(net.d, a, finish(k));
    if (rc == 0) return false;
    if (rc < 0) ckl(-rc, "falsify");
    return true;
  });


  m.def("prune_masks", [](const Net& net, int Pn, uintptr_t counts, uintptr_t ub, int ub_stride, uintptr_t sym_dead,
                          uintptr_t code, uintptr_t cnt, uintptr_t stream) {
    ckl(fa_prune_masks_launch(net.d, Pn, P<const int>(counts), P<const float>(ub), ub_stride,
                                P<const uint8_t>(sym_dead), P<uint8_t>(code), P<int>(cnt), (hipStream_t)stream),
          "prune_masks");
  });

  m.def("heuristic", [](const Net& net, int Pu, uintptr_t rows, uintptr_t lb, uintptr_t ub, int stride, uintptr_t code,
                        double q50, double qlo, double qhi, uintptr_t hnew, uintptr_t hmerged, uintptr_t hcnt,
                        uintptr_t stream) {
    ckl(fa_heuristic_launch(net.d, Pu, P<const int64_t>(rows), P<const float>(lb), P<const float>(ub), stride,
                              P<const uint8_t>(code), q50, qlo, qhi, P<uint8_t>(hnew), P<uint8_t>(hmerged),
                              P<int>(hcnt), (hipStream_t)stream),
          "heuristic");
  });

  m.def("agree", [](const Net& net, uintptr_t flat, int Pm, uintptr_t rows, uintptr_t lo, uintptr_t hi, uintptr_t pids,
                    uintptr_t dead, int S, uint32_t seed, uintptr_t agree, uintptr_t stream) {
    const int rc = fa_agree_launch(net.d, P<const float>(flat), Pm, P<const int64_t>(rows), P<const float>(lo),
                                   P<const float>(hi), P<const int64_t>(pids), P<const uint8_t>(dead), S, seed,
                                   P<int>(agree), (hipStream_t)stream);
    if (rc == 0) return false;
    if (rc < 0) ckl(-rc, "agree");
    return true;
  });

  m.def("certify", [](py::kwargs kw) {
    Kw k("certify", kw);
    auto in = [&](const char* key) { return k.need<const float>(key); };
    CertArgs a{};
    a.Nn = k.i("Nn"); a.n0 = k.i("n0"); a.V = k.i("V"); a.Pp = k.i("Pp"); a.norient = k.i("norient");
    a.Lc = in("Lc"); a.L0 = in("L0"); a.Le = in("Le"); a.Uc = in("Uc"); a.U0 = in("U0"); a.Ue = in("Ue");
    a.olb = in("olb"); a.oub = in("oub");
    a.Lcp = in("Lcp"); a.L0p = in("L0p"); a.Lep = in("Lep"); a.Ucp = in("Ucp"); a.U0p = in("U0p"); a.Uep = in("Uep");
    a.olbp = in("olbp"); a.oubp = in("oubp");
    a.xlo = in("xlo"); a.xhi = in("xhi"); a.xplo = in("xplo"); a.xphi = in("xphi");
    a.pairs = k.ptr<const int64_t>("pairs");
    a.values = k.ptr<const int64_t>("values");
    a.npa = dims(k, "pa", a.pa_idx, FA_CMAX_PA, "too many PA/RA dims");
    a.nra = dims(k, "ra", a.ra_idx, FA_MAX_RA, "too many PA/RA dims");
    a.tau = k.f("tau");
    a.shared = k.need<const uint8_t>("shared");
    a.unit = k.f("unit");
    a.gmarg = std::nextafter(k.f("gmarg"), INFINITY);
    a.gmin = k.ptr<float>("gmin"); a.tstar = k.ptr<float>("tstar");
    a.open = k.need<uint8_t>("open"); a.score = k.need<float>("score"); a.split_dim = k.need<int64_t>("split_dim");
    a.cand_x = k.need<float>("cand_x"); a.cand_xp = k.need<float>("cand_xp");
    a.cand_v = k.need<int64_t>("cand_v"); a.cand_o = k.need<int64_t>("cand_o");
    a.scores = k.ptr<float>("scores"); a.leaf = k.ptr<uint8_t>("leaf");
    ckl(fa_certify_launch(a, finish(k)), "certify");
  });

  m.def("decode", [](std::vector<int> radix, std::vector<long long> div, std::vector<int> chunk_off,
                     std::vector<float> base_lo, std::vector<float> base_hi, uintptr_t ids, int Pn,
                     uintptr_t chunk_lo, uintptr_t chunk_hi, uintptr_t lo, uintptr_t hi, uintptr_t stream) {
    const size_t n0 = radix.size();
    if (n0 == 0 || n0 > FA_DECODE_MAX_DIMS || div.size() != n0 || chunk_off.size() != n0 || base_lo.size() != n0 ||
        base_hi.size() != n0)
      throw std::invalid_argument("decode: descriptor sizes");
    DecodeDesc d{};
    d.n0 = (int)n0;
    for (size_t k = 0; k < n0; ++k) {
      if (radix[k] < 0 || (radix[k] > 0 && div[k] <= 0)) throw std::invalid_argument("decode: radix/div");
      d.radix[k] = radix[k];
      d.div[k] = div[k];
      d.chunk_off[k] = chunk_off[k];
      d.base_lo[k] = base_lo[k];
      d.base_hi[k] = base_hi[k];
    }
    ckl(fa_decode_launch(d, P<const int64_t>(ids), Pn, P<const float>(chunk_lo), P<const float>(chunk_hi),
                           P<float>(lo), P<float>(hi), (hipStream_t)stream),
          "decode");
  });
  m.def("pack_masks", [](uintptr_t src, int Pn, int N, int stride, int sel, uintptr_t out, int NB, uintptr_t hash,
                         uintptr_t stream) {
    ckl(fa_pack_masks_launch(P<const uint8_t>(src), Pn, N, stride, sel, P<uint8_t>(out), NB,
                               P<unsigned long long>(hash), (hipStream_t)stream),
          "pack_masks");
  });
  m.def("knn", [](uintptr_t X, int n, int d, int k, uintptr_t idx, uintptr_t dist, uintptr_t stream) {
    ckl(fa_knn_launch(P<const float>(X), n, d, k, P<int>(idx), P<float>(dist), (hipStream_t)stream), "knn");
  });
  m.def("actdiff", [](const Net& net, uintptr_t flat, uintptr_t x, uintptr_t xp, int npairs, uintptr_t sum_out,
                      uintptr_t stream) {
    ckl(fa_actdiff_launch(net.d, P<const float>(flat), P<const float>(x), P<const float>(xp), npairs,
                            P<float>(sum_out), (hipStream_t)stream),
          "actdiff");
  });
  m.def("trace_marker", [](int tag, uintptr_t sink, uintptr_t stream) {
    ckl(fa_trace_marker_launch(tag, P<int>(sink), (hipStream_t)stream), "trace_marker");
  });
  m.def("beta_level", [](const Net& net, py::kwargs kw) {
    Kw k("beta_level", kw);
    const BetaArgs a = beta_args(net, k);
    return fa_beta_launch(net.d, a, finish(k));
  });
  m.def("beta_level16", [](const Net& net, py::kwargs kw) {
    Kw k("beta_level16", kw);
    const BetaArgs a = beta_args(net, k);
    return fa_beta_level16_launch(net.d, a, finish(k));
  });
  m.def("beta_opt16", [](const Net& net, py::kwargs kw) {
    Kw k("beta_opt16", kw);
    BetaArgs a = beta_args(net, k);
    float* pgsum = const_cast<float*>(a.pgsum);
    float* pgn = const_cast<float*>(a.pgn);
    a.wt = a.pgsum = a.pgn = nullptr;
    return fa_beta_opt16_launch(net.d, a, pgsum, pgn, finish(k));
  });
  m.def("beta_feas", [](const Net& net, py::kwargs kw) {
    Kw k("beta_feas", kw);
    BetaArgs a = beta_args(net, k);
    const int mode = k.i("mode");
    const hipStream_t st = finish(k);
    if (mode < 0 || mode > 3) throw std::invalid_argument("beta_feas: mode must be 0..3");
    if (mode != 0 && !a.fpar) throw std::invalid_argument("beta_feas: fpar required");
    a.lookahead = a.stall = a.pgap = 0;
    a.beta_pos = a.feas = 1;
    a.split = nullptr;
    a.xstar = a.binit = a.xpstar = nullptr;
    if (mode == 0) {
      a.fpar = a.fgt = nullptr;
      return fa_beta_launch(net.d, a, st);
    }
    if (mode == 1) return fa_beta_feas16_launch(net.d, a, st);
    if (mode == 2) return fa_beta_opt16_feas_launch(net.d, a, st);
    a.iters = 0;
    return fa_beta_launch(net.d, a, st);
  });
  m.def("beta_batched_fits", [](const Net& net) { return fa_beta_opt16_fits(net.d) != 0; });
  m.def("beta_opt16_scratch", [](const Net& net, int R) { return fa_beta_opt16_scratch_floats(net.d, R); });
  m.def("beta_config", [](const Net& net) {
    int w = 0, t = 0;
    size_t b = 0;
    const int rc = fa_beta_config(net.d, &w, &t, &b);
    return py::make_tuple(rc, w, t, b);
  });
  m.def("beta_fits", [](const Net& net) {
    int w = 0, t = 0;
    size_t b = 0;
    return fa_beta_config(net.d, &w, &t, &b) == 0;
  });
  m.def("arch", []() { return std::string("gfx950"); });
  m.def("prepare_lds", [] { return fa_lds_prepare(); });
  m.def("lds_registered", [] { return (int)fa_lds_registry().size(); });
  register_bab(m);
  register_relu(m);
  register_beta(m);
  m.def("mem_stats", [] {
    const fa_mem::Stats s = fa_mem::stats();
    py::dict d;
    d["dev_cached_bytes"] = s.dev_cached_bytes;
    d["dev_live_bytes"] = s.dev_live_bytes;
    d["host_cached_bytes"] = s.host_cached_bytes;
    d["host_live_bytes"] = s.host_live_bytes;
    d["dev_mallocs"] = s.dev_mallocs;
    d["dev_hits"] = s.dev_hits;
    d["host_mallocs"] = s.host_mallocs;
    d["host_hits"] = s.host_hits;
    d["driver_frees"] = s.driver_frees;
    return d;
  });
  m.def("mem_release_cached", [] { fa_mem::release_cached(); });
  register_csv(m);
}
```

### fairify_amd/csrc/certify.hip

```cpp
#include "args.h"

struct Form {
  const float* c;
  float c0;
  float fmag;
};

__device__ __forceinline__ bool fa_is_pa(const CertArgs& a, int d) {
  for (int k = 0; k < a.npa; ++k)
    if (a.pa_idx[k] == d) return true;
  return false;
}

__device__ __forceinline__ Form fa_fold(const CertArgs& a, const float* C, float c0, int v) {
  Form f;
  f.c = C;
  float contrib = 0.f, cmag = 0.f;
  for (int k = 0; k < a.npa; ++k) {
    const float t = C[a.pa_idx[k]] * (float)a.values[v * a.npa + k];
    contrib += t;
    cmag += fabsf(t);
  }
  f.c0 = c0 + contrib;
  f.fmag = cmag;
  return f;
}

__device__ __forceinline__ void fa_pair_forms(const CertArgs& a, int n, int q, int o, Form& A, float& sA,
                                              Form& B, float& sB) {
  const int vi = (int)a.pairs[2 * q], vj = (int)a.pairs[2 * q + 1];
  const size_t ri = (size_t)n * a.V + vi, rj = (size_t)n * a.V + vj;
  if (o == 0) {
    A = fa_fold(a, a.Lc + ri * a.n0, a.L0[ri] - a.Le[ri], vi);
    sA = -1.f;
    B = fa_fold(a, a.Ucp + rj * a.n0, a.U0p[rj] + a.Uep[rj], vj);
    sB = 1.f;
  } else {
    A = fa_fold(a, a.Uc + ri * a.n0, a.U0[ri] + a.Ue[ri], vi);
    sA = 1.f;
    B = fa_fold(a, a.Lcp + rj * a.n0, a.L0p[rj] - a.Lep[rj], vj);
    sB = -1.f;
  }
}

__device__ float fa_g_at(const CertArgs& a, int n, const Form& A, float sA, const Form& B, float sB, float t,
                         float magA, float magB) {
  const float* xl = a.xlo + (size_t)n * a.n0;
  const float* xh = a.xhi + (size_t)n * a.n0;
  const float* pl = a.xplo + (size_t)n * a.n0;
  const float* ph = a.xphi + (size_t)n * a.n0;
  float val = 0.f;
  for (int i = 0; i < a.n0; ++i) {
    if (fa_is_pa(a, i)) continue;
    const float ai = sA * A.c[i];
    const float bi = sB * B.c[i];
    if (a.shared[i]) {
      const float cs = t * ai + (1.f - t) * bi;
      val += fmaxf(cs * xl[i], cs * xh[i]);
    } else {
      const float ca = t * ai, cb = (1.f - t) * bi;
      val += fmaxf(ca * xl[i], ca * xh[i]) + fmaxf(cb * pl[i], cb * ph[i]);
    }
  }
  const float A0 = sA * A.c0, B0 = sB * B.c0;
  float g = val + t * A0 + (1.f - t) * B0;
  g += a.gmarg * (t * magA + (1.f - t) * magB) + 8.f * a.unit * (magA + magB);
  return g;
}

__device__ void fa_mags(const CertArgs& a, int n, const Form& A, const Form& B, float& magA, float& magB) {
  const float* xl = a.xlo + (size_t)n * a.n0;
  const float* xh = a.xhi + (size_t)n * a.n0;
  const float* pl = a.xplo + (size_t)n * a.n0;
  const float* ph = a.xphi + (size_t)n * a.n0;
  magA = fabsf(A.c0) + A.fmag;
  magB = fabsf(B.c0) + B.fmag;
  for (int i = 0; i < a.n0; ++i) {
    if (fa_is_pa(a, i)) continue;
    magA += fabsf(A.c[i]) * fmaxf(fabsf(xl[i]), fabsf(xh[i]));
    magB += fabsf(B.c[i]) * fmaxf(fabsf(pl[i]), fabsf(ph[i]));
  }
}

#define FA_CERT_THREADS 64
template <int NM>
__device__ __forceinline__ void fa_pair_eval_one(const CertArgs& a, int n, int qq, float& gmin, float& tstar) {
  const int o = qq / a.Pp, q = qq % a.Pp;
  const int vi = (int)a.pairs[2 * q], vj = (int)a.pairs[2 * q + 1];
  {
    const size_t ri = (size_t)n * a.V + vi, rj = (size_t)n * a.V + vj;
    const bool imp = (o == 0) ? (a.olb[ri] >= 0.f || a.oubp[rj] <= 0.f) : (a.oub[ri] <= 0.f || a.olbp[rj] >= 0.f);
    if (imp) {
      gmin = -1.f;
      tstar = 0.f;
      return;
    }
  }
  Form A, B;
  float sA, sB;
  fa_pair_forms(a, n, q, o, A, sA, B, sB);
  const int n0 = a.n0;
  const float* xlp = a.xlo + (size_t)n * n0;
  const float* xhp = a.xhi + (size_t)n * n0;
  const float* plp = a.xplo + (size_t)n * n0;
  const float* php = a.xphi + (size_t)n * n0;
  float ca[NM], cb[NM], xl[NM], xh[NM], pl[NM], ph[NM];
  bool sh[NM], un[NM];
  float magA = fabsf(A.c0) + A.fmag, magB = fabsf(B.c0) + B.fmag;
#pragma unroll
  for (int i = 0; i < NM; ++i) {
    const bool v = i < n0 && !fa_is_pa(a, i);
    ca[i] = v ? sA * A.c[i] : 0.f;
    cb[i] = v ? sB * B.c[i] : 0.f;
    xl[i] = v ? xlp[i] : 0.f;
    xh[i] = v ? xhp[i] : 0.f;
    pl[i] = v ? plp[i] : 0.f;
    ph[i] = v ? php[i] : 0.f;
    sh[i] = v && a.shared[i];
    un[i] = v && !a.shared[i];
    magA += fabsf(ca[i]) * fmaxf(fabsf(xl[i]), fabsf(xh[i]));
    magB += fabsf(cb[i]) * fmaxf(fabsf(pl[i]), fabsf(ph[i]));
  }
  const float A0 = sA * A.c0, B0 = sB * B.c0;
  const float marg0 = 8.f * a.unit * (magA + magB);
  auto g_at = [&](float t) __attribute__((always_inline)) {
    float val = 0.f;
#pragma unroll
    for (int i = 0; i < NM; ++i) {
      const float cs = t * ca[i] + (1.f - t) * cb[i];
      const float c1 = t * ca[i], c2 = (1.f - t) * cb[i];
      const float vs = fmaxf(cs * xl[i], cs * xh[i]);
      const float vu = fmaxf(c1 * xl[i], c1 * xh[i]) + fmaxf(c2 * pl[i], c2 * ph[i]);
      val += sh[i] ? vs : (un[i] ? vu : 0.f);
    }
    return val + t * A0 + (1.f - t) * B0 + a.gmarg * (t * magA + (1.f - t) * magB) + marg0;
  };
  float best = g_at(0.f), bt = 0.f;
  {
    const float g1 = g_at(1.f);
    if (g1 < best) { best = g1; bt = 1.f; }
  }
  if constexpr (NM <= 16) {
#pragma unroll
    for (int i = 0; i < NM; ++i) {
      if (!sh[i]) continue;
      const float den = ca[i] - cb[i];
      if (den == 0.f) continue;
      const float t = -cb[i] / den;
      if (!(t > 0.f && t < 1.f)) continue;
      const float g = g_at(t);
      if (g < best) { best = g; bt = t; }
    }
  } else {
#pragma unroll 1
    for (int i = 0; i < n0; ++i) {
      float ai = 0.f, bi = 0.f;
      bool s_i = false;
#pragma unroll
      for (int k = 0; k < NM; ++k)
        if (k == i) { ai = ca[k]; bi = cb[k]; s_i = sh[k]; }
      if (!s_i) continue;
      const float den = ai - bi;
      if (den == 0.f) continue;
      const float t = -bi / den;
      if (!(t > 0.f && t < 1.f)) continue;
      const float g = g_at(t);
      if (g < best) { best = g; bt = t; }
    }
  }
  gmin = best;
  tstar = bt;
}

template <int NM>
__global__ void __launch_bounds__(FA_CERT_THREADS) fa_pair_eval_kernel(CertArgs a) {
  const int Q = a.Pp * a.norient;
  const int64_t idx = (int64_t)blockIdx.x * FA_CERT_THREADS + threadIdx.x;
  if (idx >= (int64_t)a.Nn * Q) return;
  float g = -INFINITY, t = 0.f;
  const int n = (int)(idx / Q);
  const int8_t st = a.status ? a.status[a.part[n]] : (int8_t)3;
  if (st == 3 || st == 4) fa_pair_eval_one<NM>(a, n, (int)(idx % Q), g, t);
  a.gmin[idx] = g;
  a.tstar[idx] = t;
}

template <int NM>
__device__ __forceinline__ void fa_pick_node(const CertArgs& a, int n, float bg, int bq, float t);

template <int NM>
__global__ void __launch_bounds__(FA_CERT_THREADS) fa_pair_pick_kernel(CertArgs a) {
  const int n = blockIdx.x * FA_CERT_THREADS + threadIdx.x;
  if (n >= a.Nn) return;
  const int Q = a.Pp * a.norient;
  float bg = -INFINITY;
  int bq = 0;
  for (int qq = 0; qq < Q; ++qq) {
    float g = a.gmin[(size_t)n * Q + qq];
    if (g != g) g = INFINITY;
    if (g > bg) { bg = g; bq = qq; }
  }
  fa_pick_node<NM>(a, n, bg, bq, a.tstar[(size_t)n * Q + bq]);
}

#ifndef FA_CERT_WPE16
#define FA_CERT_WPE16 1
#endif
template <int NM>
__global__ void __launch_bounds__(FA_CERT_THREADS) __attribute__((amdgpu_waves_per_eu(NM == 16 ? FA_CERT_WPE16 : 1)))
fa_pair_fused_kernel(CertArgs a, int QG) {
  const int Q = a.Pp * a.norient;
  const int gidx = blockIdx.x * FA_CERT_THREADS + threadIdx.x;
  const int n = gidx / QG, qq = gidx - n * QG;
  bool live = n < a.Nn && qq < Q;
  if (live && a.status) {
    const int8_t st = a.status[a.part[n]];
    live = st == 3 || st == 4;
  }
  float g = -INFINITY, t = 0.f;
  if (live) fa_pair_eval_one<NM>(a, n, qq, g, t);
  if (g != g) g = INFINITY;
  int bq = live ? qq : 0x7fffffff;
  for (int o = 1; o < QG; o <<= 1) {
    const float g2 = __shfl_xor(g, o);
    const float t2 = __shfl_xor(t, o);
    const int q2 = __shfl_xor(bq, o);
    if (g2 > g || (g2 == g && q2 < bq)) { g = g2; t = t2; bq = q2; }
  }
  if (n < a.Nn && qq == 0) fa_pick_node<NM>(a, n, g, bq == 0x7fffffff ? 0 : bq, t);
}

template <int NM>
__device__ __forceinline__ void fa_pick_node(const CertArgs& a, int n, float bg, int bq, float t) {
  if (a.skip_closed && !(bg > 0.f)) {
    a.open[n] = 0;
    a.score[n] = bg;
    if (a.leaf) a.leaf[n] = 0;
    return;
  }
  const int o = bq / a.Pp, q = bq % a.Pp;
  Form A, B;
  float sA, sB;
  fa_pair_forms(a, n, q, o, A, sA, B, sB);
  const int n0 = a.n0;
  const float* xlp = a.xlo + (size_t)n * n0;
  const float* xhp = a.xhi + (size_t)n * n0;
  const float* plp = a.xplo + (size_t)n * n0;
  const float* php = a.xphi + (size_t)n * n0;
  float* cxo = a.cand_x + (size_t)n * n0;
  float* cpo = a.cand_xp + (size_t)n * n0;
  float* sco = a.scores ? a.scores + (size_t)n * 2 * n0 : nullptr;
  float ai[NM], bi[NM], xl[NM], xh[NM], pl[NM], ph[NM];
  unsigned pam = 0u, shm = 0u;
  for (int k = 0; k < a.npa; ++k) pam |= 1u << a.pa_idx[k];
#pragma unroll
  for (int i = 0; i < NM; ++i) {
    const bool v = i < n0;
    if (v && a.shared[i]) shm |= 1u << i;
    const bool p = (pam >> i) & 1u;
    ai[i] = (v && !p) ? sA * A.c[i] : 0.f;
    bi[i] = (v && !p) ? sB * B.c[i] : 0.f;
    xl[i] = v ? xlp[i] : 0.f;
    xh[i] = v ? xhp[i] : 0.f;
    pl[i] = v ? plp[i] : 0.f;
    ph[i] = v ? php[i] : 0.f;
  }
  float bs = -1.f;
  int bd = 0;
  bool leaf = true;
#pragma unroll
  for (int i = 0; i < NM; ++i) {
    if (i >= n0) continue;
    const float wx = xh[i] - xl[i];
    const float cs = t * ai[i] + (1.f - t) * bi[i];
    float sx, cx;
    if (((shm >> i) & 1u)) {
      sx = fabsf(cs) * wx;
      cx = cs > 0.f ? xh[i] : xl[i];
    } else {
      sx = fabsf(t * ai[i]) * wx;
      cx = (t * ai[i] > 0.f) ? xh[i] : xl[i];
    }
    sx += 1e-9f * wx;
    if (((pam >> i) & 1u) || wx <= 0.f) sx = -1.f;
    if (!((pam >> i) & 1u) && wx > 0.f) leaf = false;
    if (sx > bs) { bs = sx; bd = i; }
    if (sco) sco[i] = sx;
    cxo[i] = cx;
    cpo[i] = ((shm >> i) & 1u) ? cx : (((1.f - t) * bi[i] > 0.f) ? ph[i] : pl[i]);
  }
#pragma unroll
  for (int i = 0; i < NM; ++i) {
    if (i >= n0) continue;
    float sxp = -1.f;
    if (!((shm >> i) & 1u) && !((pam >> i) & 1u)) {
      const float wxp = ph[i] - pl[i];
      if (wxp > 0.f) {
        sxp = fabsf((1.f - t) * bi[i]) * wxp + 1e-9f * wxp;
        leaf = false;
      }
    }
    if (sco) sco[n0 + i] = sxp;
    if (sxp > bs) { bs = sxp; bd = n0 + i; }
  }
  if (a.smear && sco && a.nra == 0 && n0 <= NM) {
    float acc[NM];
#pragma unroll
    for (int i = 0; i < NM; ++i) acc[i] = 0.f;
    for (int v = 0; v < a.V; ++v) {
      const float* lb = a.lay_lb + ((size_t)n * a.V + v) * a.lay_N;
      const float* ub = a.lay_ub + ((size_t)n * a.V + v) * a.lay_N;
      for (int j0 = 0; j0 < a.n1; j0 += 32) {
        unsigned msk = 0u;
#pragma unroll
        for (int k = 0; k < 32; ++k) {
          const int j = j0 + k;
          const bool jv = j < a.n1;
          const float l = jv ? lb[j] : 0.f, u = jv ? ub[j] : 0.f;
          if (l < 0.f && u > 0.f) msk |= 1u << k;
        }
        while (msk) {
          int jj[2];
#pragma unroll
          for (int k = 0; k < 2; ++k) {
            jj[k] = msk ? j0 + __builtin_ctz(msk) : -1;
            msk &= msk - 1u;
          }
          float4 w[2][NM / 4];
#pragma unroll
          for (int k = 0; k < 2; ++k) {
            const float4* wr = reinterpret_cast<const float4*>(a.W0T + (size_t)(jj[k] < 0 ? 0 : jj[k]) * NM);
#pragma unroll
            for (int i4 = 0; i4 < NM / 4; ++i4) w[k][i4] = wr[i4];
          }
#pragma unroll
          for (int k = 0; k < 2; ++k) {
            if (jj[k] < 0) break;
#pragma unroll
            for (int i4 = 0; i4 < NM / 4; ++i4) {
              acc[4 * i4] += w[k][i4].x;
              acc[4 * i4 + 1] += w[k][i4].y;
              acc[4 * i4 + 2] += w[k][i4].z;
              acc[4 * i4 + 3] += w[k][i4].w;
            }
          }
        }
      }
    }
    bs = -1.f;
    bd = 0;
#pragma unroll
    for (int i = 0; i < NM; ++i) {
      if (i >= n0) continue;
      const float wx = xh[i] - xl[i];
      float sx = acc[i] * wx + 1e-9f * wx;
      if (((pam >> i) & 1u) || wx <= 0.f) sx = -1.f;
      sco[i] = sx;
      if (sx > bs) { bs = sx; bd = i; }
    }
  }
  const int vi = (int)a.pairs[2 * q], vj = (int)a.pairs[2 * q + 1];
  for (int k = 0; k < a.npa; ++k) {
    cxo[a.pa_idx[k]] = (float)a.values[vi * a.npa + k];
    cpo[a.pa_idx[k]] = (float)a.values[vj * a.npa + k];
  }
  for (int k = 0; k < a.nra; ++k) {
    const int r = a.ra_idx[k];
    const float v = fminf(fmaxf(cpo[r], cxo[r] - a.tau), cxo[r] + a.tau);
    cpo[r] = fminf(fmaxf(v, plp[r]), php[r]);
  }
  a.open[n] = bg > 0.f ? 1 : 0;
  a.score[n] = bg;
  a.split_dim[n] = bd;
  a.cand_v[n] = q;
  a.cand_o[n] = o;
  if (a.leaf) a.leaf[n] = leaf ? 1 : 0;
}

#ifndef FA_CERT_FUSE_Q
#define FA_CERT_FUSE_Q 4
#endif

extern "C" int fa_certify_launch(CertArgs a, hipStream_t stream) {
  if (a.Nn <= 0) return 0;
  if (a.npa > FA_CMAX_PA || a.nra > FA_MAX_RA) return -3;
  const int64_t tot = (int64_t)a.Nn * a.Pp * a.norient;
  if (a.Pp * a.norient <= FA_CERT_FUSE_Q && a.n0 <= 32) {
    int QG = 1;
    while (QG < a.Pp * a.norient) QG <<= 1;
    const dim3 gn((unsigned)(((int64_t)a.Nn * QG + FA_CERT_THREADS - 1) / FA_CERT_THREADS));
    if (a.n0 <= 16) hipLaunchKernelGGL(fa_pair_fused_kernel<16>, gn, dim3(FA_CERT_THREADS), 0, stream, a, QG);
    else hipLaunchKernelGGL(fa_pair_fused_kernel<32>, gn, dim3(FA_CERT_THREADS), 0, stream, a, QG);
    return (int)hipGetLastError();
  }
  const dim3 ge((unsigned)((tot + FA_CERT_THREADS - 1) / FA_CERT_THREADS));
  if (a.n0 <= 16) hipLaunchKernelGGL(fa_pair_eval_kernel<16>, ge, dim3(FA_CERT_THREADS), 0, stream, a);
  else if (a.n0 <= 32) hipLaunchKernelGGL(fa_pair_eval_kernel<32>, ge, dim3(FA_CERT_THREADS), 0, stream, a);
  else return -4;
  const dim3 gp((a.Nn + FA_CERT_THREADS - 1) / FA_CERT_THREADS);
  if (a.n0 <= 16) hipLaunchKernelGGL(fa_pair_pick_kernel<16>, gp, dim3(FA_CERT_THREADS), 0, stream, a);
  else hipLaunchKernelGGL(fa_pair_pick_kernel<32>, gp, dim3(FA_CERT_THREADS), 0, stream, a);
  return (int)hipGetLastError();
}
```

### fairify_amd/csrc/pointfwd.h

```cpp
#pragma once
#include "args.h"

struct PointCfg {
  int w_lds[FA_MAX_LAYERS];
  int b_lds[FA_MAX_LAYERS];
  int bp_lds[FA_MAX_LAYERS];
};

template <int TM>
__device__ __forceinline__ void fa_point_layer(const NetDesc& net, const BoundArgs& a, const PointCfg& cfg,
                                               const float* smem, int l, int p0, int lane,
                                               const float (&H)[TM][4], const float (&E)[TM][4],
                                               float (&H2)[TM][4], float (&E2)[TM][4]) {
  const int col = lane & 15, grp = lane >> 4;
  const int n_in = net.dims[l], n_out = net.dims[l + 1];
  const int tin = (n_in + 15) >> 4, tout = (n_out + 15) >> 4;
  const float* sw = smem + cfg.w_lds[l];
  const float* sbp = smem + cfg.bp_lds[l];
  const bool last = l == net.n_layers - 1;
  const float gg = net.g_fwd[l];
  const float gi = net.g_one;
  const float gnext = last ? 0.f : net.g_fwd[l + 1];
  const int noff = net.neuron_off[l];
  const int p = p0 + col;
  const bool pv = p < a.R;
  const bool masked = !last && (a.dead_in || a.dead_part);
  const uint8_t* drow = nullptr;
  if (masked && pv) {
    if (a.dead_in) drow = a.dead_in + (size_t)p * net.n_hidden + noff;
    else drow = a.dead_part + (size_t)a.node_part[a.part_mod ? p % a.part_mod : p] * net.n_hidden + noff;
  }
#pragma unroll
  for (int jt = 0; jt < TM; ++jt) {
    if (jt >= tout) break;
    const float4 b4 = *reinterpret_cast<const float4*>(sbp + 16 * jt + 4 * grp);
    const float bl[4] = {b4.x, b4.y, b4.z, b4.w};
    bool forced[4] = {false, false, false, false};
    if (masked) {
#pragma unroll
      for (int i = 0; i < 4; ++i) {
        const int j = 16 * jt + 4 * grp + i;
        forced[i] = drow && j < n_out && drow[j] != 0;
      }
    }
    f32x4 Z = {0.f, 0.f, 0.f, 0.f}, Q = {0.f, 0.f, 0.f, 0.f};
    const float4* wq = reinterpret_cast<const float4*>(sw) + (size_t)jt * tin * 64 + lane;
#pragma unroll
    for (int t = 0; t < TM; ++t) {
      if (t >= tin) break;
      const float4 w4 = wq[t * 64];
      const float wv[4] = {w4.x, w4.y, w4.z, w4.w};
#pragma unroll
      for (int i = 0; i < 4; ++i) {
        Z = fa_mfma4(wv[i], H[t][i], Z);
        Q = fa_mfma4(fabsf(wv[i]), E[t][i], Q);
      }
    }
#pragma unroll
    for (int i = 0; i < 4; ++i) {
      const int j = 16 * jt + 4 * grp + i;
      const bool jv = j < n_out;
      const float b = bl[i];
      const float z = Z[i] + b;
      const float d = fmaf(gi, fabsf(z), fmaf(Q[i], 1.f + 2.f * gg, gg * fabsf(b)));
      if (last) {
        if (j == 0 && pv) {
          a.out_lb[p] = z - d;
          a.out_ub[p] = z + d;
        }
        continue;
      }
      const bool zero = !jv || forced[i] || (z + d <= 0.f);
      const float h = zero ? 0.f : fmaxf(z, 0.f);
      const float e = zero ? 0.f : d;
      H2[jt][i] = h;
      E2[jt][i] = fmaf(gnext, h, e);
    }
  }
}
```

### fairify_amd/csrc/points.hip

```cpp
#include <hip/hip_runtime.h>

#include <algorithm>
#include <map>
#include <mutex>

#include "pointfwd.h"

template <int TM>
__global__ void __launch_bounds__(FA_THREADS) __attribute__((amdgpu_waves_per_eu(TM == 7 ? 2 : 1))) fa_point_kernel(NetDesc net, BoundArgs a, PointCfg cfg) {
  extern __shared__ __attribute__((aligned(16))) float smem[];
  const int tid = threadIdx.x;
  if (a.row_open) {
    const int nw = FA_THREADS / 64;
    const int ntile = (a.R + 15) >> 4;
    int any = 0;
    for (int tile = blockIdx.x * nw + (tid >> 6); tile < ntile; tile += gridDim.x * nw) {
      const int p = tile * 16 + (tid & 15);
      any |= p < a.R && a.row_open[p % a.open_mod];
    }
    if (!__syncthreads_or(any)) return;
  }
  {
    const float4* src = reinterpret_cast<const float4*>(a.flat + net.wperm_off);
    float4* dst = reinterpret_cast<float4*>(smem);
    for (int e = tid; e < (net.wperm_floats >> 2); e += FA_THREADS) dst[e] = src[e];
    for (int l = 0; l < net.n_layers; ++l) {
      const int n_out = net.dims[l + 1];
      const float* b = a.flat + net.wperm_off + cfg.b_lds[l];
      for (int j = tid; j < ((n_out + 15) & ~15); j += FA_THREADS) smem[cfg.bp_lds[l] + j] = j < n_out ? b[j] : 0.f;
    }
  }
  __syncthreads();
  const int lane = tid & 63, col = lane & 15, grp = lane >> 4;
  const int wave = tid >> 6, nw = FA_THREADS / 64;
  const int n0 = net.dims[0];
  const int tin0 = (n0 + 15) >> 4;
  const float g0 = net.g_fwd[0];
  const int ntile = (a.R + 15) >> 4;
  for (int tile = blockIdx.x * nw + wave; tile < ntile; tile += gridDim.x * nw) {
    const int p0 = tile * 16;
    const int p = p0 + col;
    if (a.row_open && !__any(p < a.R && a.row_open[p % a.open_mod])) continue;
    float HA[TM][4], EA[TM][4], HB[TM][4], EB[TM][4];
#pragma unroll
    for (int t = 0; t < TM; ++t) {
      if (t >= tin0) break;
#pragma unroll
      for (int i = 0; i < 4; ++i) {
        const int k = 16 * t + 4 * grp + i;
        const float x = (k < n0 && p < a.R) ? a.lo[(size_t)p * n0 + k] : 0.f;
        HA[t][i] = x;
        EA[t][i] = g0 * fabsf(x);
      }
    }
    for (int l = 0; l < net.n_layers; ++l) {
      if (l & 1) fa_point_layer<TM>(net, a, cfg, smem, l, p0, lane, HB, EB, HA, EA);
      else fa_point_layer<TM>(net, a, cfg, smem, l, p0, lane, HA, EA, HB, EB);
    }
  }
}

namespace {
typedef void (*PointKernel)(NetDesc, BoundArgs, PointCfg);

PointKernel select_point(int TM) {
  if (TM <= 1) return fa_point_kernel<1>;
  if (TM <= 2) return fa_point_kernel<2>;
  if (TM <= 4) return fa_point_kernel<4>;
  if (TM <= 7) return fa_point_kernel<7>;
  if (TM <= 10) return fa_point_kernel<10>;
  return nullptr;
}

int point_cus() {
  static int cus = 0;
  static std::once_flag once;
  std::call_once(once, [] {
    int dev = 0;
    if (hipGetDevice(&dev) != hipSuccess ||
        hipDeviceGetAttribute(&cus, hipDeviceAttributeMultiprocessorCount, dev) != hipSuccess || cus <= 0)
      cus = 256;
  });
  return cus;
}
}

extern "C" int fa_point_try_launch(const NetDesc& net, BoundArgs a, hipStream_t stream) {
  if (a.R <= 0) return 1;
  int TM = 1;
  for (int l = 0; l <= net.n_layers; ++l) TM = std::max(TM, (net.dims[l] + 15) / 16);
  PointKernel k = select_point(TM);
  if (!k) return 0;
  PointCfg cfg{};
  int off = 0;
  for (int l = 0; l < net.n_layers; ++l) {
    cfg.w_lds[l] = off;
    off += ((net.dims[l] + 15) / 16) * ((net.dims[l + 1] + 15) / 16) * 256;
  }
  for (int l = 0; l < net.n_layers; ++l) {
    cfg.b_lds[l] = off;
    off += net.dims[l + 1];
  }
  if (((off + 3) & ~3) != net.wperm_floats) return -1;
  if ((size_t)net.wperm_floats * sizeof(float) > 150 * 1024) return 0;
  off = net.wperm_floats;
  for (int l = 0; l < net.n_layers; ++l) {
    cfg.bp_lds[l] = off;
    off += ((net.dims[l + 1] + 15) / 16) * 16;
  }
  const size_t bytes = (size_t)off * sizeof(float);
  static std::mutex mu;
  static std::map<std::pair<const void*, size_t>, int> occ;
  int per_cu = 0;
  {
    std::lock_guard<std::mutex> g(mu);
    const auto key = std::make_pair((const void*)k, bytes);
    auto it = occ.find(key);
    if (it == occ.end()) {
      if (!fa_lds_ok(bytes)) return -4;
      if (hipOccupancyMaxActiveBlocksPerMultiprocessor(&per_cu, k, FA_THREADS, bytes) != hipSuccess || per_cu <= 0)
        per_cu = 1;
      occ[key] = per_cu;
    } else {
      per_cu = it->second;
    }
  }
  const long long tiles = (a.R + 15) / 16;
  long long blocks = (tiles + 3) / 4;
  const long long cap = (long long)point_cus() * per_cu;
  if (blocks > cap) blocks = cap;
  hipLaunchKernelGGL(k, dim3((unsigned)blocks), dim3(FA_THREADS), bytes, stream, net, a, cfg);
  const hipError_t e = hipGetLastError();
  return e == hipSuccess ? 1 : -(int)e;
}

FA_LDS_REGISTER(FA_LDS_K(fa_point_kernel<1>), FA_LDS_K(fa_point_kernel<2>), FA_LDS_K(fa_point_kernel<4>),
                FA_LDS_K(fa_point_kernel<7>), FA_LDS_K(fa_point_kernel<10>));
```

### fairify_amd/csrc/runtime_host.h

```cpp
#pragma once

#include <hip/hip_runtime.h>
#include <pybind11/numpy.h>
#include <pybind11/pybind11.h>

#include <algorithm>
#include <cmath>
#include <cstring>
#include <stdexcept>
#include <string>
#include <vector>

#include "args.h"
#include "devmem.h"
#include "exact_host.h"

extern "C" int fa_bounds_launch(const NetDesc& net, BoundArgs args, hipStream_t stream);
extern "C" int fa_point_try_launch(const NetDesc& net, BoundArgs a, hipStream_t stream);
extern "C" int fa_set_status_launch(const int* idx, int n, int8_t* status, int8_t v, hipStream_t stream);

namespace fa_rt {

namespace py = pybind11;

inline void ck(hipError_t e, const char* what) {
  if (e != hipSuccess) throw std::runtime_error(std::string(what) + ": " + hipGetErrorString(e));
}
inline void ckl(int rc, const char* what) {
  if (rc != 0) throw std::runtime_error(std::string(what) + " launch failed, code " + std::to_string(rc));
}

inline float gamma_up(int k, double unit) {
  const double ku = (k + 2) * unit;
  return std::nextafter((float)(ku / (1.0 - ku)), INFINITY);
}

inline int grow_to(int cur, int want, int floor, int cap) {
  int n = std::max(cur, floor);
  while (n < want) n = (n > cap / 2) ? cap : n * 2;
  return std::min(n, cap);
}

inline fa_exact::ExactChecker make_exact(const NetDesc& net, const float* flat, const std::vector<int>& pa,
                                         const std::vector<int>& ra, float tau) {
  int np = 0;
  for (int l = 0; l < net.n_layers; ++l) np = std::max(np, net.b_off[l] + net.dims[l + 1]);
  std::vector<float> hf(np);
  ck(hipMemcpy(hf.data(), flat, np * sizeof(float), hipMemcpyDeviceToHost), "cp weights");
  fa_exact::ExactChecker e;
  e.n0 = net.dims[0];
  e.n_layers = net.n_layers;
  e.dims.assign(net.dims, net.dims + net.n_layers + 1);
  e.w_off.assign(net.w_off, net.w_off + net.n_layers);
  e.b_off.assign(net.b_off, net.b_off + net.n_layers);
  e.w.assign(hf.begin(), hf.end());
  e.is_pa.assign(e.n0, 0);
  e.is_ra.assign(e.n0, 0);
  for (int k : pa) e.is_pa[k] = 1;
  for (int k : ra) e.is_ra[k] = 1;
  e.tau = tau;
  return e;
}

struct LevelCounters {
  fa_mem::HostBuf hcount_buf_{true};
  LevelCounters() { hcount_buf_.ensure(4 * sizeof(int)); }
  void reset() { std::memset(hcount_buf_.p, 0, 4 * sizeof(int)); }
  int* host_ptr() { return reinterpret_cast<int*>(hcount_buf_.p); }
  int children() const { return reinterpret_cast<volatile const int*>(hcount_buf_.p)[0]; }
  int candidates() const { return reinterpret_cast<volatile const int*>(hcount_buf_.p)[1]; }
};

struct FormBufs {
  fa_mem::DevBuf<float> Lc, L0, Le, Uc, U0, Ue, olb, oub, lay_lb, lay_ub;
  void ensure(size_t rows, int n0, int n_neurons, bool with_layers) {
    Lc.ensure(rows * n0); Uc.ensure(rows * n0);
    L0.ensure(rows); Le.ensure(rows); U0.ensure(rows); Ue.ensure(rows);
    olb.ensure(rows); oub.ensure(rows);
    if (with_layers) { lay_lb.ensure(rows * n_neurons); lay_ub.ensure(rows * n_neurons); }
  }
  void fill(BoundArgs& b) const {
    b.out_lb = olb.p; b.out_ub = oub.p;
    b.Lc = Lc.p; b.L0 = L0.p; b.Le = Le.p; b.Uc = Uc.p; b.U0 = U0.p; b.Ue = Ue.p;
  }
  void fill(CrownPhaseArgs& c) const {
    c.out_lb = olb.p; c.out_ub = oub.p;
    c.Lc = Lc.p; c.L0 = L0.p; c.Le = Le.p; c.Uc = Uc.p; c.U0 = U0.p; c.Ue = Ue.p;
    c.layer_lb = lay_lb.p; c.layer_ub = lay_ub.p;
  }
};

inline void screen_points(const NetDesc& net, const float* flat, const float* pts, int rows, float* lb, float* ub,
                          hipStream_t st, const int* node_part = nullptr, int part_mod = 0,
                          const uint8_t* dead_part = nullptr, const uint8_t* row_open = nullptr, int open_mod = 0) {
  BoundArgs b{};
  b.flat = flat; b.lo = pts; b.hi = pts; b.R = rows; b.symbolic = 0;
  b.out_lb = lb; b.out_ub = ub;
  if (dead_part) { b.node_part = node_part; b.part_mod = part_mod; b.dead_part = dead_part; }
  if (row_open) { b.row_open = row_open; b.open_mod = open_mod; }
  const int prc = fa_point_try_launch(net, b, st);
  if (prc < 0) ckl(-prc, "points");
  if (prc == 0) ckl(fa_bounds_launch(net, b, st), "bounds(points)");
}

struct CandSink {
  static constexpr int kMax = 1 << 24;
  fa_mem::HostBuf cand_host_{true};
  fa_mem::HostBuf hidx_;
  fa_mem::DevBuf<int> idx_;
  int cand_alloc_ = 0;
  const int n0_;
  explicit CandSink(int n0) : n0_(n0) {}

  float* records() { return reinterpret_cast<float*>(cand_host_.p); }

  void ensure_cand(long long need, int floor) {
    if (need <= cand_alloc_) return;
    const int n = grow_to(cand_alloc_, (int)std::min<long long>(need, kMax), floor, kMax);
    cand_host_.ensure((size_t)n * (2 * n0_ + 1) * sizeof(float));
    cand_alloc_ = n;
  }

  void confirm_candidates(int n_cand, fa_exact::Witnesses& w, const fa_exact::ExactChecker* chk, py::object& confirm,
                          int8_t* status, hipStream_t st) {
    const size_t w2 = (size_t)2 * n0_;
    const std::vector<float> rec(records(), records() + (size_t)n_cand * (w2 + 1));
    const std::vector<int> newly = fa_exact::select_witnesses(
        rec.data(), n_cand, w, chk,
        [&](const std::vector<int>& slots, const std::vector<float>& pairs, const std::vector<int>& parts) {
          py::gil_scoped_acquire gil;
          const int na = (int)slots.size();
          py::array_t<float> abuf({na, 2 * n0_});
          py::array_t<int> aparts(na);
          std::memcpy(abuf.mutable_data(), pairs.data(), sizeof(float) * pairs.size());
          std::memcpy(aparts.mutable_data(), parts.data(), sizeof(int) * parts.size());
          py::array_t<bool> res = confirm(aparts, abuf).cast<py::array_t<bool>>();
          if (res.size() != na) throw std::runtime_error("candidate confirmation: answer count mismatch");
          return std::vector<char>(res.data(), res.data() + na);
        });
    if (newly.empty()) return;
    idx_.ensure(newly.size());
    hidx_.ensure(newly.size() * sizeof(int));
    std::memcpy(hidx_.p, newly.data(), newly.size() * sizeof(int));
    ck(hipMemcpyAsync(idx_.p, hidx_.p, newly.size() * sizeof(int), hipMemcpyHostToDevice, st), "cp idx");
    ckl(fa_set_status_launch(idx_.p, (int)newly.size(), status, 1, st), "set_status");
  }
};

}
```

Measured before the change: 279,900.

## Compact open nodes on device so point screening and split touch only survivors

The certify kernel now appends still-open nodes to a device index list with a per-sub-batch counter. The point-forward screening and the split kernel read that count and process only the compacted rows, exiting early for blocks past the count instead of scanning every node. Candidate and score buffers are written in compacted order. This adds atomic counter traffic, counter clearing in settle and init, and an extra indirection per node, and requires the point kernel path to be available.

```diff
diff --git a/fairify_amd/csrc/args.h b/fairify_amd/csrc/args.h
--- a/fairify_amd/csrc/args.h
+++ b/fairify_amd/csrc/args.h
@@ -37,6 +37,8 @@
   int skip_signdef;
   const uint8_t* row_open;
   int open_mod;
+  const int* row_count;
+  const int* row_node;
   const int8_t* phase_in;
   uint8_t* infeas;
 };
@@ -170,6 +172,8 @@
   int lay_N;
   const float* W0T;
   int n1;
+  int* open_idx;
+  int* open_count;
 };
 
 struct SettleArgs {
@@ -189,6 +193,8 @@
   int max_open;
   EscSteps esc;
   int* done;
+  int* open_counts;
+  int n_open_counts;
 };
 
 struct SplitArgs {
@@ -230,6 +236,8 @@
   int* cand_count;
   int cand_cap;
   SettleArgs settle;
+  const int* open_idx;
+  const int* open_count;
 };
 
 struct BabInitArgs {
@@ -243,6 +251,8 @@
   int ra_idx[FA_MAX_RA];
   float tau;
   int* counters;
+  int* open_counts;
+  int n_open_counts;
   int* pbudget;
   uint8_t* prob;
   int budget;
diff --git a/fairify_amd/csrc/bab.hip b/fairify_amd/csrc/bab.hip
--- a/fairify_amd/csrc/bab.hip
+++ b/fairify_amd/csrc/bab.hip
@@ -71,6 +71,10 @@
   s.counters_next[1] = 0;
 }
 
+__device__ __forceinline__ void fa_settle_open_counts(const SettleArgs& s, int i, int nth) {
+  for (; i < s.n_open_counts; i += nth) s.open_counts[i] = 0;
+}
+
 __device__ __forceinline__ void fa_settle_part(const SettleArgs& s, int p) {
   const int8_t st = s.status[p];
   if (st == ST_STOPPING) {
@@ -129,25 +133,39 @@
   float pe[FA_SPLIT_NB][4];
   int8_t st[FA_SPLIT_NB];
   uint8_t open[FA_SPLIT_NB], leaf[FA_SPLIT_NB];
+  int node[FA_SPLIT_NB];
   int last;
 };
 
-__device__ __forceinline__ void fa_split_fetch(const SplitArgs& a, FaSplitLds& sh, int nb) {
+__device__ __forceinline__ int fa_split_fetch(const SplitArgs& a, FaSplitLds& sh, int nb) {
+  int cnt = a.Nn;
+  if (a.open_idx) cnt = min(max(*a.open_count, 0), a.Nn);
   if (threadIdx.x >= nb && threadIdx.x < FA_SPLIT_NB) sh.plan[threadIdx.x] = FaSplitPlan{0ull, 0ull, 0, 0, 0, 0, -1};
   if (threadIdx.x < nb) {
     const int t = threadIdx.x;
-    const int n = blockIdx.x * nb + t;
+    const int e = blockIdx.x * nb + t;
     uint8_t op = 0;
-    int p = 0;
-    if (n < a.Nn) {
-      op = a.open[n];
+    int p = 0, n = -1;
+    if (e < cnt) {
+      if (a.open_idx) {
+        n = a.open_idx[e];
+        op = 1;
+        sh.pe[t][0] = a.pe_lb[2 * e];
+        sh.pe[t][1] = a.pe_ub[2 * e];
+        sh.pe[t][2] = a.pe_lb[2 * e + 1];
+        sh.pe[t][3] = a.pe_ub[2 * e + 1];
+      } else {
+        n = e;
+        op = a.open[e];
+        sh.pe[t][0] = a.pe_lb[e];
+        sh.pe[t][1] = a.pe_ub[e];
+        sh.pe[t][2] = a.pe_lb[a.Nn + e];
+        sh.pe[t][3] = a.pe_ub[a.Nn + e];
+      }
       p = a.part[n];
-      sh.leaf[t] = a.leaf[n];
-      sh.pe[t][0] = a.pe_lb[n];
-      sh.pe[t][1] = a.pe_ub[n];
-      sh.pe[t][2] = a.pe_lb[a.Nn + n];
-      sh.pe[t][3] = a.pe_ub[a.Nn + n];
-    }
+      sh.leaf[t] = a.leaf[e];
+    }
+    sh.node[t] = n;
     sh.open[t] = op;
     sh.part[t] = p;
     if (op) {
@@ -158,6 +176,7 @@
     }
   }
   __syncthreads();
+  return cnt;
 }
 
 __device__ __forceinline__ void fa_split_reserve(const SplitArgs& a, FaSplitLds& sh) {
@@ -201,6 +220,7 @@
     if (sh.last) {
       __threadfence();
       if (threadIdx.x == 0) fa_settle_counters(a.settle);
+      fa_settle_open_counts(a.settle, threadIdx.x, blockDim.x);
       for (int p = threadIdx.x; p < a.settle.P; p += blockDim.x) fa_settle_part(a.settle, p);
       if (threadIdx.x == 0) *a.settle.done = 0;
     }
@@ -230,9 +250,10 @@
 }
 
 template <int W>
-__device__ __forceinline__ void fa_split_write_inner(const SplitArgs& a, const FaSplitPlan& pl, int n, int p, int slot,
-                                                     int off, int li) {
+__device__ __forceinline__ void fa_split_write_inner(const SplitArgs& a, const FaSplitPlan& pl, int n, int e, int p,
+                                                     int slot, int off, int li) {
   const int n0 = a.n0;
+  const int cs = a.open_idx ? 2 * n0 : n0;
   const float* xl = a.xlo + (size_t)n * n0;
   const float* xh = a.xhi + (size_t)n * n0;
   const float* xpl = a.relaxed ? a.xplo + (size_t)n * n0 : xl;
@@ -241,8 +262,8 @@
     if (slot < a.cand_cap) {
       float* cbuf = a.cand_buf + (size_t)slot * (2 * n0 + 1);
       for (int d = li; d < 2 * n0 + 1; d += W)
-        cbuf[d] = d < n0 ? a.cand_x[(size_t)n * n0 + d]
-                         : (d < 2 * n0 ? a.cand_xp[(size_t)n * n0 + d - n0] : __int_as_float(p));
+        cbuf[d] = d < n0 ? a.cand_x[(size_t)e * cs + d]
+                         : (d < 2 * n0 ? a.cand_xp[(size_t)e * cs + d - n0] : __int_as_float(p));
     }
   }
   if (pl.nchild == 0) return;
@@ -290,13 +311,17 @@
   const int n0 = a.n0;
   const int npair = a.norient * a.Pp;
   const int nb = FA_SPLIT_WAVES * npw;
-  fa_split_fetch(a, sh, nb);
+  if (fa_split_fetch(a, sh, nb) <= (int)blockIdx.x * nb) {
+    fa_split_settle_tail(a, sh);
+    return;
+  }
   for (int i = 0; i < npw; ++i) {
     const int loc = wave * npw + i;
-    const int n = blockIdx.x * nb + loc;
+    const int e = blockIdx.x * nb + loc;
+    const int n = sh.node[loc];
     FaSplitPlan pl{0ull, 0ull, 0, 0, 0, 0, -1};
     do {
-      if (n >= a.Nn || !sh.open[loc]) break;
+      if (n < 0 || !sh.open[loc]) break;
       const int p = sh.part[loc];
       const int8_t s0 = sh.st[loc];
       if (s0 != ST_RUNNING && s0 != ST_STOPPING) break;
@@ -312,7 +337,7 @@
         const float lbp = sh.pe[loc][2], ubp = sh.pe[loc][3];
         pl.ncand = ((lbx < 0.f && ubp > 0.f) || (ubx > 0.f && lbp < 0.f)) ? 1 : 0;
       }
-      const float* sc = a.scores + (size_t)n * 2 * n0;
+      const float* sc = a.scores + (size_t)e * 2 * n0;
       int mreq = 1;
       {
         const int mmax = a.m < FA_MAX_SPLIT ? a.m : FA_MAX_SPLIT;
@@ -370,7 +395,8 @@
   fa_split_reserve(a, sh);
   for (int i = 0; i < npw; ++i) {
     const int loc = wave * npw + i;
-    const int n = blockIdx.x * nb + loc;
+    const int e = blockIdx.x * nb + loc;
+    const int n = sh.node[loc];
     const FaSplitPlan pl = sh.plan[loc];
     if (pl.ncand == 0 && pl.nchild == 0) continue;
     const int p = sh.part[loc];
@@ -388,7 +414,7 @@
       }
       continue;
     }
-    fa_split_write_inner<64>(a, pl, n, p, sh.cand_off[loc], sh.child_off[loc], lane);
+    fa_split_write_inner<64>(a, pl, n, e, p, sh.cand_off[loc], sh.child_off[loc], lane);
   }
   fa_split_settle_tail(a, sh);
 }
@@ -404,12 +430,16 @@
   const int npair = a.norient * a.Pp;
   const int nb = FA_SPLIT_WAVES * FA_SPLIT_GPW * npp;
   const int mmax = a.m < FA_MAX_SPLIT ? a.m : FA_MAX_SPLIT;
-  fa_split_fetch(a, sh, nb);
+  if (fa_split_fetch(a, sh, nb) <= (int)blockIdx.x * nb) {
+    fa_split_settle_tail(a, sh);
+    return;
+  }
   for (int i = 0; i < npp; ++i) {
     const int loc = (wave * npp + i) * FA_SPLIT_GPW + grp;
-    const int n = blockIdx.x * nb + loc;
+    const int e = blockIdx.x * nb + loc;
+    const int n = sh.node[loc];
     FaSplitPlan pl{0ull, 0ull, 0, 0, 0, 0, -1};
-    bool act = n < a.Nn && sh.open[loc];
+    bool act = n >= 0 && sh.open[loc];
     const int p = sh.part[loc];
     if (act) {
       const int8_t s0 = sh.st[loc];
@@ -434,7 +464,7 @@
       pl.ncand = ((lbx < 0.f && ubp > 0.f) || (ubx > 0.f && lbp < 0.f)) ? 1 : 0;
       const int w = sh.ws[loc];
       while (mreq < mmax && ((long long)w << (mreq + 1)) <= (long long)a.target) ++mreq;
-      const float* sc = a.scores + (size_t)n * 2 * n0;
+      const float* sc = a.scores + (size_t)e * 2 * n0;
       if (d0 < 2 * n0) s0v = sc[d0];
       if (d1 < 2 * n0) s1v = sc[d1];
       if (!(s0v > -0.5f)) s0v = -1.f;
@@ -500,7 +530,8 @@
   fa_split_reserve(a, sh);
   for (int i = 0; i < npp; ++i) {
     const int loc = (wave * npp + i) * FA_SPLIT_GPW + grp;
-    const int n = blockIdx.x * nb + loc;
+    const int e = blockIdx.x * nb + loc;
+    const int n = sh.node[loc];
     const FaSplitPlan pl = sh.plan[loc];
     const bool any = pl.ncand != 0 || pl.nchild != 0;
     if (!__ballot(any)) continue;
@@ -516,7 +547,7 @@
         slot0 += __popcll(bm);
       }
     }
-    if (any && !pl.leaf) fa_split_write_inner<16>(a, pl, n, p, sh.cand_off[loc], sh.child_off[loc], gl);
+    if (any && !pl.leaf) fa_split_write_inner<16>(a, pl, n, e, p, sh.cand_off[loc], sh.child_off[loc], gl);
   }
   fa_split_settle_tail(a, sh);
 }
@@ -552,6 +583,7 @@
     }
   }
   if (tid < 5) a.counters[tid] = 0;
+  for (int i = tid; i < a.n_open_counts; i += nth) a.open_counts[i] = 0;
 }
 
 __global__ void fa_bab_finish_kernel(int P, const int8_t* status, const int* nodes, const int* open_left, int* out) {
@@ -572,6 +604,7 @@
 __global__ void fa_settle_kernel(SettleArgs s) {
   const int p = blockIdx.x * FA_THREADS + threadIdx.x;
   if (p == 0) fa_settle_counters(s);
+  fa_settle_open_counts(s, p, gridDim.x * FA_THREADS);
   if (p < s.P) fa_settle_part(s, p);
 }
 
@@ -583,6 +616,7 @@
 extern "C" int fa_split_launch(SplitArgs a, hipStream_t stream) {
   if (a.Nn <= 0) return 0;
   if (a.nra > FA_MAX_RA || a.npa > FA_CMAX_PA || a.n0 > 64) return -3;
+  if ((a.open_idx != nullptr) != (a.open_count != nullptr)) return -3;
   if (2 * a.n0 <= 32) {
     const char* e = getenv("FAIRIFY_SPLIT_GROUPS");
     if (!(e && *e == '0')) {
diff --git a/fairify_amd/csrc/bab_runtime.cpp b/fairify_amd/csrc/bab_runtime.cpp
--- a/fairify_amd/csrc/bab_runtime.cpp
+++ b/fairify_amd/csrc/bab_runtime.cpp
@@ -6,6 +6,7 @@
 #include <algorithm>
 #include <chrono>
 #include <cmath>
+#include <cstdio>
 #include <cstring>
 #include <stdexcept>
 #include <utility>
@@ -16,6 +17,8 @@
 namespace py = pybind11;
 
 extern "C" int fa_certify_launch(CertArgs a, hipStream_t stream);
+extern "C" int fa_cert_compact_ok(int n0, int Pp, int norient);
+extern "C" int fa_point_fits(const NetDesc& net);
 extern "C" int fa_split_launch(SplitArgs a, hipStream_t stream);
 extern "C" int fa_mark_unknown_launch(const int* part, int n, int8_t* status, hipStream_t stream);
 extern "C" int fa_settle_launch(SettleArgs s, hipStream_t stream);
@@ -65,6 +68,16 @@
     return !(e && e[0] == '0');
   }();
   return v;
+}
+
+bool tail_compact() {
+  const char* e = getenv("FAIRIFY_TAIL_COMPACT");
+  return !(e && e[0] == '0');
+}
+
+bool tail_stats() {
+  const char* e = getenv("FAIRIFY_TAIL_STATS");
+  return e && e[0] == '1';
 }
 
 }
@@ -122,6 +135,11 @@
     scores_.ensure((size_t)batch_ * 2 * n0_);
     pe_lb_.ensure(2 * (size_t)batch_);
     pe_ub_.ensure(2 * (size_t)batch_);
+    compact_ok_ = fa_cert_compact_ok(n0_, Pp_, norient_) != 0 && fa_point_fits(net_) != 0;
+    if (compact_ok_) {
+      open_idx_.ensure(batch_);
+      open_cnt_.ensure(64);
+    }
     sink_.ensure_cand(cand_cap_, kCandFloor);
     counters_.ensure(5);
     exact_ = fa_rt::make_exact(net_, flat_, pa_, relaxed_ ? ra_ : std::vector<int>(), tau_);
@@ -168,6 +186,10 @@
       prob_.ensure(P);
     }
     int slot = 0;
+    const bool compact = compact_ok_ && tail_compact();
+    const bool diag = tail_stats();
+    long long diag_open = 0;
+    std::vector<uint8_t> diag_buf;
     const int8_t* hstatus = status0.data();
     std::vector<int> run;
     for (int p = 0; p < P; ++p)
@@ -204,6 +226,7 @@
       for (int k = 0; k < ia.nra; ++k) ia.ra_idx[k] = ra_[k];
       ia.tau = tau_;
       ia.counters = counters_.p;
+      ia.open_counts = open_cnt_.p; ia.n_open_counts = (int)open_cnt_.n;
       ia.pbudget = inline_esc ? pbudget_.p : nullptr;
       ia.prob = inline_esc ? prob_.p : nullptr;
       ia.budget = budget;
@@ -236,6 +259,14 @@
       se.pbudget = inline_esc ? pbudget_.p : nullptr; se.prob = inline_esc ? prob_.p : nullptr;
       se.budget2 = budget2; se.max_open = max_w; se.esc = esc;
       se.done = counters_.p + 4;
+      const int nsub = (n_in + batch_ - 1) / batch_;
+      if (compact) {
+        if ((size_t)nsub > open_cnt_.n) {
+          open_cnt_.ensure(nsub);
+          ck(hipMemsetAsync(open_cnt_.p, 0, open_cnt_.n * sizeof(int), st), "clear open counters");
+        }
+        se.open_counts = open_cnt_.p; se.n_open_counts = nsub;
+      }
       bool settled = false;
       for (int s = 0; s < n_in; s += batch_) {
         const int nb = std::min(batch_, n_in - s);
@@ -265,17 +296,39 @@
         c.gmin = gmin_.p; c.tstar = tstar_.p;
         c.open = open_.p; c.score = score_.p; c.split_dim = split_.p;
         c.cand_x = cand_.p; c.cand_xp = cand_.p + (size_t)nb * n0_;
+        int* ocount = nullptr;
+        if (compact) {
+          ocount = open_cnt_.p + s / batch_;
+          c.open_idx = open_idx_.p; c.open_count = ocount;
+          c.cand_xp = cand_.p + n0_;
+        }
         c.cand_v = cv_.p; c.cand_o = co_.p;
         c.scores = scores_.p; c.leaf = leaf_.p;
-        if (cert_skip_closed()) { c.skip_closed = 1; c.status = status_.p; c.part = bpart; }
+        if (compact || cert_skip_closed()) { c.skip_closed = 1; c.status = status_.p; c.part = bpart; }
         if (smear_ && !relaxed_) {
           c.smear = 1;
           c.lay_lb = fx.lay_lb.p; c.lay_ub = fx.lay_ub.p; c.lay_N = net_.n_neurons;
           c.W0T = w0t_.p; c.n1 = net_.dims[1];
         }
         ckl(fa_certify_launch(c, st), "certify");
-        fa_rt::screen_points(net_, flat_, cand_.p, 2 * nb, pe_lb_.p, pe_ub_.p, st, bpart, nb,
-                             (const uint8_t*)dead_part, point_skip_closed() ? open_.p : nullptr, nb);
+        if (diag) {
+          ck(hipStreamSynchronize(st), "sync (tail stats)");
+          if (compact) {
+            int cnt = 0;
+            ck(hipMemcpy(&cnt, ocount, sizeof(int), hipMemcpyDeviceToHost), "cp (tail stats)");
+            diag_open += cnt;
+          } else {
+            diag_buf.resize(nb);
+            ck(hipMemcpy(diag_buf.data(), open_.p, nb, hipMemcpyDeviceToHost), "cp (tail stats)");
+            for (int k = 0; k < nb; ++k) diag_open += diag_buf[k] ? 1 : 0;
+          }
+        }
+        if (compact)
+          fa_rt::screen_points(net_, flat_, cand_.p, 2 * nb, pe_lb_.p, pe_ub_.p, st, bpart, 0,
+                               (const uint8_t*)dead_part, nullptr, 0, ocount, open_idx_.p);
+        else
+          fa_rt::screen_points(net_, flat_, cand_.p, 2 * nb, pe_lb_.p, pe_ub_.p, st, bpart, nb,
+                               (const uint8_t*)dead_part, point_skip_closed() ? open_.p : nullptr, nb);
         SplitArgs sa{};
         sa.Nn = nb; sa.n0 = n0_; sa.relaxed = relaxed_ ? 1 : 0; sa.nra = relaxed_ ? (int)ra_.size() : 0;
         for (int k = 0; k < sa.nra; ++k) sa.ra_idx[k] = ra_[k];
@@ -283,6 +336,7 @@
         sa.xlo = blo; sa.xhi = bhi; sa.xplo = bplo; sa.xphi = bphi; sa.part = bpart;
         sa.open = open_.p; sa.leaf = leaf_.p; sa.scores = scores_.p;
         sa.cand_x = c.cand_x; sa.cand_xp = c.cand_xp; sa.pe_lb = pe_lb_.p; sa.pe_ub = pe_ub_.p;
+        sa.open_idx = c.open_idx; sa.open_count = c.open_count;
         sa.olb = c.olb; sa.oub = c.oub; sa.olbp = c.olbp; sa.oubp = c.oubp;
         sa.pairs = pairs_.p; sa.values = vals_i_.p; sa.npa = npa_;
         for (int k = 0; k < npa_; ++k) sa.pa_idx[k] = pa_[k];
@@ -347,6 +401,15 @@
     stats["nodes"] = total_nodes;
     stats["time"] = el;
     stats["timed_out"] = timed_out;
+    if (diag) {
+      stats["tail_open"] = diag_open;
+      stats["tail_nodes"] = total_nodes;
+      stats["tail_compact"] = compact;
+      std::string dims;
+      for (int l = 0; l <= net_.n_layers; ++l) dims += (l ? "," : "") + std::to_string(net_.dims[l]);
+      std::fprintf(stderr, "fairify tail-stats dims=%s compact=%d levels=%d open=%lld nodes=%lld\n", dims.c_str(),
+                   compact ? 1 : 0, levels, diag_open, total_nodes);
+    }
     py::array_t<int64_t> ax({P, n0_}), axp({P, n0_});
     std::memcpy(ax.mutable_data(), wit.cex_x.data(), sizeof(int64_t) * wit.cex_x.size());
     std::memcpy(axp.mutable_data(), wit.cex_xp.data(), sizeof(int64_t) * wit.cex_xp.size());
@@ -428,6 +491,7 @@
   bool crown_ = false;
   int refine_ = 0;
   bool smear_ = false;
+  bool compact_ok_ = false;
   bool fuse_settle_ = fuse_settle();
   int split_target_ = 256;
   int n0_ = 0, npa_ = 0, V_ = 0, Pp_ = 0, norient_ = 1;
@@ -441,6 +505,7 @@
   DevBuf<float> gmin_, tstar_, score_, cand_, scores_, pe_lb_, pe_ub_;
   DevBuf<uint8_t> open_, leaf_;
   DevBuf<int64_t> split_, cv_, co_;
+  DevBuf<int> open_idx_, open_cnt_;
   DevBuf<int> counters_, nodes_, open_left_, lvl_open_, nodes_start_, prev_start_, out_, pbudget_;
   DevBuf<int8_t> status_;
   DevBuf<uint8_t> prob_;
diff --git a/fairify_amd/csrc/bindings.cpp b/fairify_amd/csrc/bindings.cpp
--- a/fairify_amd/csrc/bindings.cpp
+++ b/fairify_amd/csrc/bindings.cpp
@@ -25,6 +25,7 @@
 extern "C" int fa_count_level_launch(CountArgs a, hipStream_t stream);
 extern "C" int fa_ascent_launch(const NetDesc& net, AscentArgs a, hipStream_t stream);
 extern "C" int fa_certify_launch(CertArgs a, hipStream_t stream);
+extern "C" int fa_cert_compact_ok(int n0, int Pp, int norient);
 extern "C" int fa_falsify_launch(const NetDesc& net, FalsifyArgs a, hipStream_t stream);
 extern "C" int fa_prune_masks_launch(const NetDesc& net, int P, const int* counts, const float* ub, int ub_stride,
                                      const uint8_t* sym_dead, uint8_t* code, int* cnt, hipStream_t stream);
@@ -323,9 +324,16 @@
     a.row_open = k.ptr<const uint8_t>("row_open");
     a.open_mod = k.i("open_mod", 0);
     if (a.row_open && a.open_mod <= 0) throw std::invalid_argument("point_bounds: row_open needs open_mod > 0");
+    a.row_count = k.ptr<const int>("row_count");
+    a.row_node = k.ptr<const int>("row_node");
+    a.node_part = k.ptr<const int>("node_part");
+    a.dead_part = k.ptr<const uint8_t>("dead_part");
+    if ((a.dead_part != nullptr) != (a.node_part != nullptr) || (a.row_node && !a.row_count))
+      throw std::invalid_argument("point_bounds: dead_part needs node_part, row_node needs row_count");
     const hipStream_t stream = finish(k);
     const int rc = fa_point_try_launch(net.d, a, stream);
     if (rc < 0) ckl(-rc, "point_bounds");
+    if (rc == 0 && a.row_count) throw std::invalid_argument("point_bounds: row_count needs the point kernel");
     if (rc == 0) ckl(fa_bounds_launch(net.d, a, stream), "point_bounds(ibp)");
   });
 
@@ -536,6 +544,19 @@
     a.cand_x = k.need<float>("cand_x"); a.cand_xp = k.need<float>("cand_xp");
     a.cand_v = k.need<int64_t>("cand_v"); a.cand_o = k.need<int64_t>("cand_o");
     a.scores = k.ptr<float>("scores"); a.leaf = k.ptr<uint8_t>("leaf");
+    a.skip_closed = k.i("skip_closed", 0);
+    a.status = k.ptr<const int8_t>("status"); a.part = k.ptr<const int>("part");
+    if ((a.status != nullptr) != (a.part != nullptr)) throw std::invalid_argument("certify: status needs part");
+    a.smear = k.i("smear", 0);
+    a.lay_lb = k.ptr<const float>("lay_lb"); a.lay_ub = k.ptr<const float>("lay_ub"); a.lay_N = k.i("lay_N", 0);
+    a.W0T = k.ptr<const float>("W0T"); a.n1 = k.i("n1", 0);
+    if (a.smear && (!a.lay_lb || !a.lay_ub || !a.W0T || a.n1 <= 0 || a.lay_N < a.n1))
+      throw std::invalid_argument("certify: smear needs lay_lb, lay_ub, lay_N, W0T and n1");
+    a.open_idx = k.ptr<int>("open_idx"); a.open_count = k.ptr<int>("open_count");
+    if ((a.open_idx != nullptr) != (a.open_count != nullptr))
+      throw std::invalid_argument("certify: open_idx and open_count come together");
+    if (a.open_idx && !fa_cert_compact_ok(a.n0, a.Pp, a.norient))
+      throw std::invalid_argument("certify: compact mode needs the fused path (Pp * norient <= 4, n0 <= 32)");
     ckl(fa_certify_launch(a, finish(k)), "certify");
   });
 
diff --git a/fairify_amd/csrc/certify.hip b/fairify_amd/csrc/certify.hip
--- a/fairify_amd/csrc/certify.hip
+++ b/fairify_amd/csrc/certify.hip
@@ -186,7 +186,7 @@
 }
 
 template <int NM>
-__device__ __forceinline__ void fa_pick_node(const CertArgs& a, int n, float bg, int bq, float t);
+__device__ __forceinline__ void fa_pick_node(const CertArgs& a, int n, int s, float bg, int bq, float t);
 
 template <int NM>
 __global__ void __launch_bounds__(FA_CERT_THREADS) fa_pair_pick_kernel(CertArgs a) {
@@ -200,17 +200,22 @@
     if (g != g) g = INFINITY;
     if (g > bg) { bg = g; bq = qq; }
   }
-  fa_pick_node<NM>(a, n, bg, bq, a.tstar[(size_t)n * Q + bq]);
+  fa_pick_node<NM>(a, n, n, bg, bq, a.tstar[(size_t)n * Q + bq]);
 }
 
 #ifndef FA_CERT_WPE16
 #define FA_CERT_WPE16 1
 #endif
-template <int NM>
-__global__ void __launch_bounds__(FA_CERT_THREADS) __attribute__((amdgpu_waves_per_eu(NM == 16 ? FA_CERT_WPE16 : 1)))
+#ifndef FA_CERT_CTHREADS
+#define FA_CERT_CTHREADS 128
+#endif
+template <int NM, bool COMPACT>
+__global__ void __launch_bounds__(COMPACT ? FA_CERT_CTHREADS : FA_CERT_THREADS)
+    __attribute__((amdgpu_waves_per_eu(NM == 16 ? FA_CERT_WPE16 : 1)))
 fa_pair_fused_kernel(CertArgs a, int QG) {
+  constexpr int NT = COMPACT ? FA_CERT_CTHREADS : FA_CERT_THREADS;
   const int Q = a.Pp * a.norient;
-  const int gidx = blockIdx.x * FA_CERT_THREADS + threadIdx.x;
+  const int gidx = blockIdx.x * NT + threadIdx.x;
   const int n = gidx / QG, qq = gidx - n * QG;
   bool live = n < a.Nn && qq < Q;
   if (live && a.status) {
@@ -227,15 +232,47 @@
     const int q2 = __shfl_xor(bq, o);
     if (g2 > g || (g2 == g && q2 < bq)) { g = g2; t = t2; bq = q2; }
   }
-  if (n < a.Nn && qq == 0) fa_pick_node<NM>(a, n, g, bq == 0x7fffffff ? 0 : bq, t);
+  if (bq == 0x7fffffff) bq = 0;
+  if constexpr (!COMPACT) {
+    if (n < a.Nn && qq == 0) fa_pick_node<NM>(a, n, n, g, bq, t);
+  } else {
+    constexpr int NW = NT / 64;
+    __shared__ int s_wcnt[NW], s_base, s_n[NT], s_q[NT];
+    __shared__ float s_g[NT], s_t[NT];
+    const int lane = threadIdx.x & 63, wave = threadIdx.x >> 6;
+    const bool op = n < a.Nn && qq == 0 && g > 0.f;
+    const unsigned long long bm = __ballot(op);
+    if (lane == 0) s_wcnt[wave] = __popcll(bm);
+    __syncthreads();
+    int before = 0, cnt = 0;
+#pragma unroll
+    for (int w = 0; w < NW; ++w) {
+      const int c = s_wcnt[w];
+      if (w < wave) before += c;
+      cnt += c;
+    }
+    if (cnt == 0) return;
+    if (threadIdx.x == 0) s_base = atomicAdd(a.open_count, cnt);
+    if (op) {
+      const int k = before + __popcll(bm & ((1ull << lane) - 1ull));
+      s_n[k] = n; s_g[k] = g; s_q[k] = bq; s_t[k] = t;
+    }
+    __syncthreads();
+    const int k = threadIdx.x;
+    const int slot = s_base + k;
+    if (k < cnt && slot < a.Nn) {
+      a.open_idx[slot] = s_n[k];
+      fa_pick_node<NM>(a, s_n[k], slot, s_g[k], s_q[k], s_t[k]);
+    }
+  }
 }
 
 template <int NM>
-__device__ __forceinline__ void fa_pick_node(const CertArgs& a, int n, float bg, int bq, float t) {
+__device__ __forceinline__ void fa_pick_node(const CertArgs& a, int n, int s, float bg, int bq, float t) {
   if (a.skip_closed && !(bg > 0.f)) {
-    a.open[n] = 0;
-    a.score[n] = bg;
-    if (a.leaf) a.leaf[n] = 0;
+    a.open[s] = 0;
+    a.score[s] = bg;
+    if (a.leaf) a.leaf[s] = 0;
     return;
   }
   const int o = bq / a.Pp, q = bq % a.Pp;
@@ -247,9 +284,10 @@
   const float* xhp = a.xhi + (size_t)n * n0;
   const float* plp = a.xplo + (size_t)n * n0;
   const float* php = a.xphi + (size_t)n * n0;
-  float* cxo = a.cand_x + (size_t)n * n0;
-  float* cpo = a.cand_xp + (size_t)n * n0;
-  float* sco = a.scores ? a.scores + (size_t)n * 2 * n0 : nullptr;
+  const int cs = a.open_idx ? 2 * n0 : n0;
+  float* cxo = a.cand_x + (size_t)s * cs;
+  float* cpo = a.cand_xp + (size_t)s * cs;
+  float* sco = a.scores ? a.scores + (size_t)s * 2 * n0 : nullptr;
   float ai[NM], bi[NM], xl[NM], xh[NM], pl[NM], ph[NM];
   unsigned pam = 0u, shm = 0u;
   for (int k = 0; k < a.npa; ++k) pam |= 1u << a.pa_idx[k];
@@ -369,17 +407,21 @@
     const float v = fminf(fmaxf(cpo[r], cxo[r] - a.tau), cxo[r] + a.tau);
     cpo[r] = fminf(fmaxf(v, plp[r]), php[r]);
   }
-  a.open[n] = bg > 0.f ? 1 : 0;
-  a.score[n] = bg;
-  a.split_dim[n] = bd;
-  a.cand_v[n] = q;
-  a.cand_o[n] = o;
-  if (a.leaf) a.leaf[n] = leaf ? 1 : 0;
+  a.open[s] = bg > 0.f ? 1 : 0;
+  a.score[s] = bg;
+  a.split_dim[s] = bd;
+  a.cand_v[s] = q;
+  a.cand_o[s] = o;
+  if (a.leaf) a.leaf[s] = leaf ? 1 : 0;
 }
 
 #ifndef FA_CERT_FUSE_Q
 #define FA_CERT_FUSE_Q 4
 #endif
+
+extern "C" int fa_cert_compact_ok(int n0, int Pp, int norient) {
+  return Pp * norient <= FA_CERT_FUSE_Q && n0 <= 32;
+}
 
 extern "C" int fa_certify_launch(CertArgs a, hipStream_t stream) {
   if (a.Nn <= 0) return 0;
@@ -388,11 +430,19 @@
   if (a.Pp * a.norient <= FA_CERT_FUSE_Q && a.n0 <= 32) {
     int QG = 1;
     while (QG < a.Pp * a.norient) QG <<= 1;
+    if (a.open_idx) {
+      if (!a.open_count || !a.scores || !a.leaf) return -5;
+      const dim3 gc((unsigned)(((int64_t)a.Nn * QG + FA_CERT_CTHREADS - 1) / FA_CERT_CTHREADS));
+      if (a.n0 <= 16) hipLaunchKernelGGL((fa_pair_fused_kernel<16, true>), gc, dim3(FA_CERT_CTHREADS), 0, stream, a, QG);
+      else hipLaunchKernelGGL((fa_pair_fused_kernel<32, true>), gc, dim3(FA_CERT_CTHREADS), 0, stream, a, QG);
+      return (int)hipGetLastError();
+    }
     const dim3 gn((unsigned)(((int64_t)a.Nn * QG + FA_CERT_THREADS - 1) / FA_CERT_THREADS));
-    if (a.n0 <= 16) hipLaunchKernelGGL(fa_pair_fused_kernel<16>, gn, dim3(FA_CERT_THREADS), 0, stream, a, QG);
-    else hipLaunchKernelGGL(fa_pair_fused_kernel<32>, gn, dim3(FA_CERT_THREADS), 0, stream, a, QG);
+    if (a.n0 <= 16) hipLaunchKernelGGL((fa_pair_fused_kernel<16, false>), gn, dim3(FA_CERT_THREADS), 0, stream, a, QG);
+    else hipLaunchKernelGGL((fa_pair_fused_kernel<32, false>), gn, dim3(FA_CERT_THREADS), 0, stream, a, QG);
     return (int)hipGetLastError();
   }
+  if (a.open_idx) return -5;
   const dim3 ge((unsigned)((tot + FA_CERT_THREADS - 1) / FA_CERT_THREADS));
   if (a.n0 <= 16) hipLaunchKernelGGL(fa_pair_eval_kernel<16>, ge, dim3(FA_CERT_THREADS), 0, stream, a);
   else if (a.n0 <= 32) hipLaunchKernelGGL(fa_pair_eval_kernel<32>, ge, dim3(FA_CERT_THREADS), 0, stream, a);
diff --git a/fairify_amd/csrc/pointfwd.h b/fairify_amd/csrc/pointfwd.h
--- a/fairify_amd/csrc/pointfwd.h
+++ b/fairify_amd/csrc/pointfwd.h
@@ -11,7 +11,8 @@
 __device__ __forceinline__ void fa_point_layer(const NetDesc& net, const BoundArgs& a, const PointCfg& cfg,
                                                const float* smem, int l, int p0, int lane,
                                                const float (&H)[TM][4], const float (&E)[TM][4],
-                                               float (&H2)[TM][4], float (&E2)[TM][4]) {
+                                               float (&H2)[TM][4], float (&E2)[TM][4], int rows = -1) {
+  const int R = rows < 0 ? a.R : rows;
   const int col = lane & 15, grp = lane >> 4;
   const int n_in = net.dims[l], n_out = net.dims[l + 1];
   const int tin = (n_in + 15) >> 4, tout = (n_out + 15) >> 4;
@@ -23,12 +24,15 @@
   const float gnext = last ? 0.f : net.g_fwd[l + 1];
   const int noff = net.neuron_off[l];
   const int p = p0 + col;
-  const bool pv = p < a.R;
+  const bool pv = p < R;
   const bool masked = !last && (a.dead_in || a.dead_part);
   const uint8_t* drow = nullptr;
   if (masked && pv) {
     if (a.dead_in) drow = a.dead_in + (size_t)p * net.n_hidden + noff;
-    else drow = a.dead_part + (size_t)a.node_part[a.part_mod ? p % a.part_mod : p] * net.n_hidden + noff;
+    else {
+      const int node = a.row_node ? a.row_node[p >> 1] : (a.part_mod ? p % a.part_mod : p);
+      drow = a.dead_part + (size_t)a.node_part[node] * net.n_hidden + noff;
+    }
   }
 #pragma unroll
   for (int jt = 0; jt < TM; ++jt) {
diff --git a/fairify_amd/csrc/points.hip b/fairify_amd/csrc/points.hip
--- a/fairify_amd/csrc/points.hip
+++ b/fairify_amd/csrc/points.hip
@@ -10,13 +10,19 @@
 __global__ void __launch_bounds__(FA_THREADS) __attribute__((amdgpu_waves_per_eu(TM == 7 ? 2 : 1))) fa_point_kernel(NetDesc net, BoundArgs a, PointCfg cfg) {
   extern __shared__ __attribute__((aligned(16))) float smem[];
   const int tid = threadIdx.x;
+  int R = a.R;
+  if (a.row_count) {
+    const int c = *a.row_count;
+    R = min(R, 2 * max(c, 0));
+    if (blockIdx.x * (FA_THREADS / 64) >= ((R + 15) >> 4)) return;
+  }
   if (a.row_open) {
     const int nw = FA_THREADS / 64;
-    const int ntile = (a.R + 15) >> 4;
+    const int ntile = (R + 15) >> 4;
     int any = 0;
     for (int tile = blockIdx.x * nw + (tid >> 6); tile < ntile; tile += gridDim.x * nw) {
       const int p = tile * 16 + (tid & 15);
-      any |= p < a.R && a.row_open[p % a.open_mod];
+      any |= p < R && a.row_open[p % a.open_mod];
     }
     if (!__syncthreads_or(any)) return;
   }
@@ -36,11 +42,11 @@
   const int n0 = net.dims[0];
   const int tin0 = (n0 + 15) >> 4;
   const float g0 = net.g_fwd[0];
-  const int ntile = (a.R + 15) >> 4;
+  const int ntile = (R + 15) >> 4;
   for (int tile = blockIdx.x * nw + wave; tile < ntile; tile += gridDim.x * nw) {
     const int p0 = tile * 16;
     const int p = p0 + col;
-    if (a.row_open && !__any(p < a.R && a.row_open[p % a.open_mod])) continue;
+    if (a.row_open && !__any(p < R && a.row_open[p % a.open_mod])) continue;
     float HA[TM][4], EA[TM][4], HB[TM][4], EB[TM][4];
 #pragma unroll
     for (int t = 0; t < TM; ++t) {
@@ -48,14 +54,14 @@
 #pragma unroll
       for (int i = 0; i < 4; ++i) {
         const int k = 16 * t + 4 * grp + i;
-        const float x = (k < n0 && p < a.R) ? a.lo[(size_t)p * n0 + k] : 0.f;
+        const float x = (k < n0 && p < R) ? a.lo[(size_t)p * n0 + k] : 0.f;
         HA[t][i] = x;
         EA[t][i] = g0 * fabsf(x);
       }
     }
     for (int l = 0; l < net.n_layers; ++l) {
-      if (l & 1) fa_point_layer<TM>(net, a, cfg, smem, l, p0, lane, HB, EB, HA, EA);
-      else fa_point_layer<TM>(net, a, cfg, smem, l, p0, lane, HA, EA, HB, EB);
+      if (l & 1) fa_point_layer<TM>(net, a, cfg, smem, l, p0, lane, HB, EB, HA, EA, R);
+      else fa_point_layer<TM>(net, a, cfg, smem, l, p0, lane, HA, EA, HB, EB, R);
     }
   }
 }
@@ -83,6 +89,12 @@
   });
   return cus;
 }
+}
+
+extern "C" int fa_point_fits(const NetDesc& net) {
+  int TM = 1;
+  for (int l = 0; l <= net.n_layers; ++l) TM = std::max(TM, (net.dims[l] + 15) / 16);
+  return select_point(TM) != nullptr && (size_t)net.wperm_floats * sizeof(float) <= 150 * 1024;
 }
 
 extern "C" int fa_point_try_launch(const NetDesc& net, BoundArgs a, hipStream_t stream) {
diff --git a/fairify_amd/csrc/runtime_host.h b/fairify_amd/csrc/runtime_host.h
--- a/fairify_amd/csrc/runtime_host.h
+++ b/fairify_amd/csrc/runtime_host.h
@@ -92,14 +92,18 @@
 
 inline void screen_points(const NetDesc& net, const float* flat, const float* pts, int rows, float* lb, float* ub,
                           hipStream_t st, const int* node_part = nullptr, int part_mod = 0,
-                          const uint8_t* dead_part = nullptr, const uint8_t* row_open = nullptr, int open_mod = 0) {
+                          const uint8_t* dead_part = nullptr, const uint8_t* row_open = nullptr, int open_mod = 0,
+                          const int* row_count = nullptr, const int* row_node = nullptr) {
   BoundArgs b{};
   b.flat = flat; b.lo = pts; b.hi = pts; b.R = rows; b.symbolic = 0;
   b.out_lb = lb; b.out_ub = ub;
   if (dead_part) { b.node_part = node_part; b.part_mod = part_mod; b.dead_part = dead_part; }
   if (row_open) { b.row_open = row_open; b.open_mod = open_mod; }
+  b.row_count = row_count;
+  if (row_count && dead_part) b.row_node = row_node;
   const int prc = fa_point_try_launch(net, b, st);
   if (prc < 0) ckl(-prc, "points");
+  if (prc == 0 && row_count) throw std::runtime_error("screen_points: a device row count needs the point kernel");
   if (prc == 0) ckl(fa_bounds_launch(net, b, st), "bounds(points)");
 }
 
```

After: 278,800 (median of 2 runs). About the same (-0.4%).
